# alibaba/EasyParallelLibrary

Hardware: AMD Instinct MI355X
Metric: samples_per_sec (higher is better)
Workload: dtype bf16; 1 GPU; model=bert-large, global_batch=128, seq_len=512, parallelism=dp1

## Files before the change

### csrc/bindings.hip

```cpp

#include <hip/hip_runtime.h>
#include <torch/extension.h>
#include <ATen/hip/impl/HIPStreamMasqueradingAsCUDA.h>

#include <cstdint>

namespace epl {
void register_comm(py::module& m);
}

extern "C" {
void epl_fused_adamw(float*, unsigned short*, const void*, bool, float*,
                     float*, int64_t, float, float, float, float, float, int,
                     float, hipStream_t);
void epl_lamb_phase1(const float*, const void*, bool, float*, float*, float*,
                     const int*, float*, float*, int64_t, float, float, float,
                     float, int, float, hipStream_t);
void epl_lamb_phase2(float*, unsigned short*, const float*, const int*,
                     const float*, int64_t, float, hipStream_t);
void epl_layer_norm_fwd(void*, const void*, const void*, void*, const void*,
                        const void*, float*, float*, int64_t, int64_t, float,
                        bool, hipStream_t);
void epl_layer_norm_bwd(void*, float*, float*, const void*, const void*,
                        const void*, const float*, const float*, float*,
                        float*, int64_t, int64_t, int64_t, bool,
                        hipStream_t);
void epl_bias_gelu_fwd(void*, const void*, const void*, int64_t, int64_t,
                       bool, hipStream_t);
void epl_bias_gelu_bwd(void*, float*, const void*, const void*, const void*,
                       float*, int64_t, int64_t, int64_t, bool,
                       hipStream_t);
void epl_ce_rowstats(const void*, const int64_t*, float*, float*, float*,
                     int64_t, int64_t, int64_t, int64_t, bool, hipStream_t);
void epl_ce_backward(void*, const void*, const int64_t*, const float*,
                     const float*, const float*, int64_t, int64_t, int64_t,
                     int64_t, float, bool, hipStream_t);
void epl_scale(void*, int64_t, float, bool, hipStream_t);
void epl_f32_to_bf16(unsigned short*, const float*, int64_t, hipStream_t);
void epl_bf16_to_f32(float*, const unsigned short*, int64_t, hipStream_t);
void epl_sqnorm(const void*, int64_t, float*, bool, hipStream_t);
void epl_colsum(void*, const void*, float*, int64_t, int64_t, int64_t,
                bool, hipStream_t);
void run_mfma_probe(const unsigned short*, const unsigned short*, float*,
                    hipStream_t);
void epl_moe_dispatch_fwd(void*, const void*, const int64_t*,
                          const int64_t*, const int64_t*, int64_t, int64_t,
                          int64_t, hipStream_t);
void epl_moe_dispatch_bwd(void*, const void*, const int64_t*,
                          const int64_t*, const int64_t*, int64_t, int64_t,
                          int64_t, int64_t, hipStream_t);
void epl_moe_combine_fwd(void*, const void*, const float*, const int64_t*,
                         const int64_t*, const int64_t*, int64_t, int64_t,
                         int64_t, int64_t, hipStream_t);
void epl_moe_combine_bwd(void*, float*, const void*, const void*,
                         const float*, const int64_t*, const int64_t*,
                         const int64_t*, int64_t, int64_t, int64_t,
                         hipStream_t);
void epl_attn_fwd(const void*, const void*, const void*, void*, float*,
                  int64_t, int64_t, float, bool, int64_t, int64_t,
                  const int64_t*,
                  const int64_t*, unsigned int*, int64_t,
                  unsigned long long, int, float, hipStream_t);
void epl_attn_bwd(const void*, const void*, const void*, const void*,
                  const void*, const float*, float*, void*, void*, void*,
                  int64_t, int64_t, float, bool, int64_t, const int64_t*,
                  const int64_t*, const int64_t*, const int64_t*, int,
                  const unsigned int*, int64_t, float, int64_t,
                  const float*, hipStream_t);
}

namespace {

hipStream_t cur_stream() {
  return c10::hip::getCurrentHIPStreamMasqueradingAsCUDA().stream();
}

void check(const at::Tensor& t, at::ScalarType dtype, const char* name) {
  TORCH_CHECK(t.is_cuda(), name, " must be a device tensor");
  TORCH_CHECK(t.is_contiguous(), name, " must be contiguous");
  TORCH_CHECK(t.scalar_type() == dtype, name, " has dtype ", t.scalar_type(),
              ", expected ", dtype);
}

bool is_bf16(const at::Tensor& t) {
  TORCH_CHECK(t.scalar_type() == at::kBFloat16 || t.scalar_type() == at::kFloat,
              "expected bf16 or fp32, got ", t.scalar_type());
  return t.scalar_type() == at::kBFloat16;
}

void fused_adamw(at::Tensor master, c10::optional<at::Tensor> param_bf16,
                 at::Tensor grad, at::Tensor m, at::Tensor v, double lr,
                 double beta1, double beta2, double eps, double weight_decay,
                 int64_t step, double inv_scale) {
  check(master, at::kFloat, "master");
  check(m, at::kFloat, "m");
  check(v, at::kFloat, "v");
  const bool gbf = is_bf16(grad);
  unsigned short* pb = nullptr;
  if (param_bf16.has_value()) {
    check(*param_bf16, at::kBFloat16, "param_bf16");
    TORCH_CHECK(param_bf16->numel() == master.numel());
    pb = reinterpret_cast<unsigned short*>(param_bf16->data_ptr());
  }
  const int64_t n = master.numel();
  TORCH_CHECK(grad.numel() == n && m.numel() == n && v.numel() == n,
              "arena size mismatch");
  epl_fused_adamw(master.data_ptr<float>(), pb, grad.data_ptr(), gbf,
                  m.data_ptr<float>(), v.data_ptr<float>(), n, (float)lr,
                  (float)beta1, (float)beta2, (float)eps, (float)weight_decay,
                  (int)step, (float)inv_scale, cur_stream());
}

void lamb_phase1(at::Tensor master, at::Tensor grad, at::Tensor m,
                 at::Tensor v, at::Tensor update, at::Tensor chunk_of,
                 at::Tensor wnorm_sq, at::Tensor unorm_sq, double beta1,
                 double beta2, double eps, double weight_decay, int64_t step,
                 double inv_scale) {
  check(master, at::kFloat, "master");
  check(update, at::kFloat, "update");
  check(chunk_of, at::kInt, "chunk_of");
  const bool gbf = is_bf16(grad);
  epl_lamb_phase1(master.data_ptr<float>(), grad.data_ptr(), gbf,
                  m.data_ptr<float>(), v.data_ptr<float>(),
                  update.data_ptr<float>(), chunk_of.data_ptr<int>(),
                  wnorm_sq.data_ptr<float>(), unorm_sq.data_ptr<float>(),
                  master.numel(), (float)beta1, (float)beta2, (float)eps,
                  (float)weight_decay, (int)step, (float)inv_scale,
                  cur_stream());
}

void lamb_phase2(at::Tensor master, c10::optional<at::Tensor> param_bf16,
                 at::Tensor update, at::Tensor chunk_of, at::Tensor ratio,
                 double lr) {
  check(master, at::kFloat, "master");
  unsigned short* pb = nullptr;
  if (param_bf16.has_value())
    pb = reinterpret_cast<unsigned short*>(param_bf16->data_ptr());
  epl_lamb_phase2(master.data_ptr<float>(), pb, update.data_ptr<float>(),
                  chunk_of.data_ptr<int>(), ratio.data_ptr<float>(),
                  master.numel(), (float)lr, cur_stream());
}

void layer_norm_fwd(at::Tensor out, at::Tensor x,
                    c10::optional<at::Tensor> res,
                    c10::optional<at::Tensor> sum_out, at::Tensor gamma,
                    at::Tensor beta, at::Tensor mean, at::Tensor rstd,
                    double eps) {
  const bool bf16 = is_bf16(x);
  const int64_t cols = x.size(-1);
  const int64_t rows = x.numel() / cols;
  TORCH_CHECK(!bf16 || cols % 8 == 0, "bf16 LayerNorm needs cols % 8 == 0");
  check(mean, at::kFloat, "mean");
  check(rstd, at::kFloat, "rstd");
  const void* res_p = nullptr;
  void* sum_p = nullptr;
  if (res.has_value()) {
    TORCH_CHECK(sum_out.has_value(),
                "fused residual LayerNorm needs sum_out");
    TORCH_CHECK(res->numel() == x.numel() && sum_out->numel() == x.numel());
    res_p = res->data_ptr();
    sum_p = sum_out->data_ptr();
  }
  epl_layer_norm_fwd(out.data_ptr(), x.data_ptr(), res_p, sum_p,
                     gamma.data_ptr(), beta.data_ptr(),
                     mean.data_ptr<float>(), rstd.data_ptr<float>(), rows,
                     cols, (float)eps, bf16, cur_stream());
}

void layer_norm_bwd(at::Tensor dx, at::Tensor dgamma, at::Tensor dbeta,
                    at::Tensor dy, at::Tensor x, at::Tensor gamma,
                    at::Tensor mean, at::Tensor rstd) {
  const bool bf16 = is_bf16(x);
  const int64_t cols = x.size(-1);
  const int64_t rows = x.numel() / cols;
  TORCH_CHECK(!bf16 || cols % 8 == 0, "bf16 LayerNorm needs cols % 8 == 0");
  TORCH_CHECK((size_t)cols * 2 * sizeof(float) <= 128 * 1024,
              "LayerNorm backward supports cols <= 16384");
  check(dgamma, at::kFloat, "dgamma");
  check(dbeta, at::kFloat, "dbeta");
  float* dgp = nullptr;
  float* dbp = nullptr;
  at::Tensor ws;
  const bool fast = bf16 && cols % 8 == 0 && cols <= 2048;
  int64_t nparts = 0;
  if (fast) {
    const int64_t wave_rows = (rows + 3) / 4;
    nparts = (wave_rows < 1024 ? wave_rows : 1024) * 4;
    ws = at::empty({2, nparts, cols}, dgamma.options());
    dgp = ws.data_ptr<float>();
    dbp = dgp + nparts * cols;
  }
  epl_layer_norm_bwd(dx.data_ptr(), dgamma.data_ptr<float>(),
                     dbeta.data_ptr<float>(), dy.data_ptr(), x.data_ptr(),
                     gamma.data_ptr(), mean.data_ptr<float>(),
                     rstd.data_ptr<float>(), dgp, dbp, nparts, rows, cols,
                     bf16, cur_stream());
}

void bias_gelu_fwd(at::Tensor out, at::Tensor x, at::Tensor bias) {
  const bool bf16 = is_bf16(x);
  const int64_t cols = x.size(-1);
  const int64_t rows = x.numel() / cols;
  TORCH_CHECK(!bf16 || cols % 8 == 0, "bf16 bias_gelu needs cols % 8 == 0");
  epl_bias_gelu_fwd(out.data_ptr(), x.data_ptr(), bias.data_ptr(), rows, cols,
                    bf16, cur_stream());
}

void bias_gelu_bwd(at::Tensor dx, at::Tensor dbias, at::Tensor dy,
                   at::Tensor x, at::Tensor bias) {
  const bool bf16 = is_bf16(x);
  const int64_t cols = x.size(-1);
  const int64_t rows = x.numel() / cols;
  TORCH_CHECK(!bf16 || cols % 8 == 0, "bf16 bias_gelu needs cols % 8 == 0");
  TORCH_CHECK((size_t)cols * sizeof(float) <= 128 * 1024,
              "bias_gelu backward supports cols <= 32768");
  check(dbias, at::kFloat, "dbias");
  float* dbp = nullptr;
  int64_t nwaves = 0;
  at::Tensor ws;
  if (bf16 && cols % 512 == 0) {
    const int64_t segs = cols / 512;
    int64_t per_seg = rows < 1024 ? rows : 1024;
    per_seg = (per_seg + 3) / 4 * 4;
    nwaves = segs * per_seg;
    ws = at::empty({nwaves, 512}, dbias.options());
    dbp = ws.data_ptr<float>();
  }
  epl_bias_gelu_bwd(dx.data_ptr(), dbias.data_ptr<float>(), dy.data_ptr(),
                    x.data_ptr(), bias.data_ptr(), dbp, nwaves, rows, cols,
                    bf16, cur_stream());
}

void ce_rowstats(at::Tensor logits, at::Tensor targets, at::Tensor row_max,
                 at::Tensor row_sumexp, at::Tensor target_logit,
                 int64_t vocab_begin, int64_t ignore_index) {
  const bool bf16 = is_bf16(logits);
  const int64_t cols = logits.size(-1);
  const int64_t rows = logits.numel() / cols;
  check(targets, at::kLong, "targets");
  epl_ce_rowstats(logits.data_ptr(), targets.data_ptr<int64_t>(),
                  row_max.data_ptr<float>(), row_sumexp.data_ptr<float>(),
                  target_logit.data_ptr<float>(), rows, cols, vocab_begin,
                  ignore_index, bf16, cur_stream());
}

void ce_backward(at::Tensor dlogits, at::Tensor logits, at::Tensor targets,
                 at::Tensor gmax, at::Tensor gsumexp, at::Tensor dloss,
                 int64_t vocab_begin, int64_t ignore_index, double scale) {
  const bool bf16 = is_bf16(logits);
  const int64_t cols = logits.size(-1);
  const int64_t rows = logits.numel() / cols;
  epl_ce_backward(dlogits.data_ptr(), logits.data_ptr(),
                  targets.data_ptr<int64_t>(), gmax.data_ptr<float>(),
                  gsumexp.data_ptr<float>(), dloss.data_ptr<float>(), rows,
                  cols, vocab_begin, ignore_index, (float)scale, bf16,
                  cur_stream());
}

void scale_(at::Tensor t, double s) {
  const bool bf16 = is_bf16(t);
  epl_scale(t.data_ptr(), t.numel(), (float)s, bf16, cur_stream());
}

void f32_to_bf16(at::Tensor dst, at::Tensor src) {
  check(dst, at::kBFloat16, "dst");
  check(src, at::kFloat, "src");
  TORCH_CHECK(dst.numel() == src.numel());
  epl_f32_to_bf16(reinterpret_cast<unsigned short*>(dst.data_ptr()),
                  src.data_ptr<float>(), src.numel(), cur_stream());
}

void bf16_to_f32(at::Tensor dst, at::Tensor src) {
  check(dst, at::kFloat, "dst");
  check(src, at::kBFloat16, "src");
  TORCH_CHECK(dst.numel() == src.numel());
  epl_bf16_to_f32(dst.data_ptr<float>(),
                  reinterpret_cast<unsigned short*>(src.data_ptr()),
                  src.numel(), cur_stream());
}

static void attn_strides(const at::Tensor& t, int64_t* out3,
                         const char* name) {
  TORCH_CHECK(t.dim() == 4 && (t.size(3) == 64 || t.size(3) == 128), name,
              " must be [B,H,S,64|128]");
  TORCH_CHECK(t.stride(3) == 1, name, " last dim must be contiguous");
  TORCH_CHECK(t.stride(2) % 8 == 0 && t.stride(1) % 8 == 0,
              name, " row strides must be 16-byte aligned");
  out3[0] = t.stride(0);
  out3[1] = t.stride(1);
  out3[2] = t.stride(2);
}

void attn_fwd(at::Tensor q, at::Tensor k, at::Tensor v, at::Tensor out,
              at::Tensor lse, double scale, bool causal,
              c10::optional<at::Tensor> drop_mask, int64_t seed,
              int64_t drop_thresh, double inv_keep) {
  TORCH_CHECK(q.is_cuda() && q.scalar_type() == at::kBFloat16);
  int64_t in_s[3], o_s[3], tmp[3];
  attn_strides(q, in_s, "q");
  attn_strides(k, tmp, "k");
  TORCH_CHECK(tmp[0] == in_s[0] && tmp[1] == in_s[1] && tmp[2] == in_s[2],
              "q/k/v must share strides");
  attn_strides(v, tmp, "v");
  TORCH_CHECK(tmp[0] == in_s[0] && tmp[1] == in_s[1] && tmp[2] == in_s[2],
              "q/k/v must share strides");
  attn_strides(out, o_s, "out");
  check(lse, at::kFloat, "lse");
  const int64_t heads = q.size(1);
  const int64_t seq = q.size(2);
  const int64_t head_dim = q.size(3);
  const int64_t bh = q.size(0) * heads;
  unsigned int* mptr = nullptr;
  int64_t mask_w = (seq + 31) / 32;
  if (drop_mask.has_value()) {
    check(*drop_mask, at::kInt, "drop_mask");
    TORCH_CHECK(drop_mask->numel() == bh * seq * mask_w,
                "drop_mask size mismatch");
    TORCH_CHECK(drop_thresh > 0 && drop_thresh < 256, "drop_thresh range");
    mptr = reinterpret_cast<unsigned int*>(drop_mask->data_ptr());
  }
  epl_attn_fwd(q.data_ptr(), k.data_ptr(), v.data_ptr(), out.data_ptr(),
               lse.data_ptr<float>(), bh, seq, (float)scale, causal, heads,
               head_dim, in_s, o_s, mptr, mask_w,
               (unsigned long long)seed, (int)drop_thresh,
               (float)inv_keep, cur_stream());
}

void attn_bwd(at::Tensor q, at::Tensor k, at::Tensor v, at::Tensor out,
              at::Tensor dout, at::Tensor lse, at::Tensor delta_ws,
              at::Tensor dq, at::Tensor dk, at::Tensor dv, double scale,
              bool causal, bool split_dkdv,
              c10::optional<at::Tensor> drop_mask, double inv_keep,
              c10::optional<at::Tensor> dlse) {
  int64_t in_s[3], o_s[3], do_s[3], g_s[3], tmp[3];
  attn_strides(q, in_s, "q");
  attn_strides(out, o_s, "out");
  attn_strides(dout, do_s, "dout");
  attn_strides(dq, g_s, "dq");
  attn_strides(dk, tmp, "dk");
  TORCH_CHECK(tmp[0] == g_s[0] && tmp[1] == g_s[1] && tmp[2] == g_s[2],
              "dq/dk/dv must share strides");
  attn_strides(dv, tmp, "dv");
  TORCH_CHECK(tmp[0] == g_s[0] && tmp[1] == g_s[1] && tmp[2] == g_s[2],
              "dq/dk/dv must share strides");
  const int64_t heads = q.size(1);
  const int64_t seq = q.size(2);
  const int64_t bh = q.size(0) * heads;
  check(delta_ws, at::kFloat, "delta_ws");
  const unsigned int* mptr = nullptr;
  int64_t mask_w = (seq + 31) / 32;
  if (drop_mask.has_value()) {
    check(*drop_mask, at::kInt, "drop_mask");
    mptr = reinterpret_cast<const unsigned int*>(drop_mask->data_ptr());
  }
  const float* dlse_ptr = nullptr;
  if (dlse.has_value()) {
    check(*dlse, at::kFloat, "dlse");
    TORCH_CHECK(dlse->numel() == bh * seq, "dlse size mismatch");
    dlse_ptr = dlse->data_ptr<float>();
  }
  epl_attn_bwd(q.data_ptr(), k.data_ptr(), v.data_ptr(), out.data_ptr(),
               dout.data_ptr(), lse.data_ptr<float>(),
               delta_ws.data_ptr<float>(), dq.data_ptr(), dk.data_ptr(),
               dv.data_ptr(), bh, seq, (float)scale, causal, heads, in_s,
               o_s, do_s, g_s, split_dkdv ? 1 : 0, mptr, mask_w,
               (float)inv_keep, q.size(3), dlse_ptr, cur_stream());
}

void mfma_probe(at::Tensor A, at::Tensor B, at::Tensor D) {
  check(A, at::kBFloat16, "A");
  check(B, at::kBFloat16, "B");
  check(D, at::kFloat, "D");
  run_mfma_probe(reinterpret_cast<const unsigned short*>(A.data_ptr()),
                 reinterpret_cast<const unsigned short*>(B.data_ptr()),
                 D.data_ptr<float>(), cur_stream());
}

static void check_idx(const at::Tensor& t, const char* name) {
  TORCH_CHECK(t.is_cuda() && t.is_contiguous() &&
              t.scalar_type() == at::kLong, name,
              " must be a contiguous int64 device tensor");
}

void moe_dispatch_fwd(at::Tensor disp, at::Tensor x, at::Tensor fe,
                      at::Tensor pos, at::Tensor ft, int64_t cap) {
  check(disp, at::kBFloat16, "disp");
  check(x, at::kBFloat16, "x");
  check_idx(fe, "fe"); check_idx(pos, "pos"); check_idx(ft, "ft");
  const int64_t hidden = x.size(-1);
  TORCH_CHECK(hidden % 8 == 0, "hidden % 8");
  epl_moe_dispatch_fwd(disp.data_ptr(), x.data_ptr(),
                       fe.data_ptr<int64_t>(), pos.data_ptr<int64_t>(),
                       ft.data_ptr<int64_t>(), fe.numel(), hidden, cap,
                       cur_stream());
}

void moe_dispatch_bwd(at::Tensor dx, at::Tensor ddisp, at::Tensor fe,
                      at::Tensor pos, at::Tensor inv, int64_t k,
                      int64_t cap) {
  check(dx, at::kBFloat16, "dx");
  check(ddisp, at::kBFloat16, "ddisp");
  check_idx(fe, "fe"); check_idx(pos, "pos"); check_idx(inv, "inv");
  const int64_t hidden = dx.size(-1);
  epl_moe_dispatch_bwd(dx.data_ptr(), ddisp.data_ptr(),
                       fe.data_ptr<int64_t>(), pos.data_ptr<int64_t>(),
                       inv.data_ptr<int64_t>(), dx.numel() / hidden, k,
                       hidden, cap, cur_stream());
}

void moe_combine_fwd(at::Tensor out, at::Tensor h, at::Tensor fw,
                     at::Tensor fe, at::Tensor pos, at::Tensor inv,
                     int64_t k, int64_t cap) {
  check(out, at::kBFloat16, "out");
  check(h, at::kBFloat16, "h");
  check(fw, at::kFloat, "fw");
  check_idx(fe, "fe"); check_idx(pos, "pos"); check_idx(inv, "inv");
  const int64_t hidden = out.size(-1);
  epl_moe_combine_fwd(out.data_ptr(), h.data_ptr(), fw.data_ptr<float>(),
                      fe.data_ptr<int64_t>(), pos.data_ptr<int64_t>(),
                      inv.data_ptr<int64_t>(), out.numel() / hidden, k,
                      hidden, cap, cur_stream());
}

void moe_combine_bwd(at::Tensor dh, at::Tensor dfw, at::Tensor dout,
                     at::Tensor h, at::Tensor fw, at::Tensor fe,
                     at::Tensor pos, at::Tensor ft, int64_t cap) {
  check(dh, at::kBFloat16, "dh");
  check(dout, at::kBFloat16, "dout");
  check(h, at::kBFloat16, "h");
  check(fw, at::kFloat, "fw");
  check(dfw, at::kFloat, "dfw");
  check_idx(fe, "fe"); check_idx(pos, "pos"); check_idx(ft, "ft");
  const int64_t hidden = dh.size(-1);
  epl_moe_combine_bwd(dh.data_ptr(), dfw.data_ptr<float>(),
                      dout.data_ptr(), h.data_ptr(), fw.data_ptr<float>(),
                      fe.data_ptr<int64_t>(), pos.data_ptr<int64_t>(),
                      ft.data_ptr<int64_t>(), fe.numel(), hidden, cap,
                      cur_stream());
}

void colsum(at::Tensor dy, at::Tensor db, at::Tensor partial) {
  const bool bf16 = is_bf16(dy);
  TORCH_CHECK(dy.is_cuda() && dy.is_contiguous() && dy.dim() == 2,
              "dy must be a contiguous 2-D device tensor");
  const int64_t rows = dy.size(0), cols = dy.size(1);
  TORCH_CHECK(cols % 8 == 0, "cols must be a multiple of 8");
  TORCH_CHECK(db.numel() == cols && db.scalar_type() == dy.scalar_type());
  const int64_t stripes = partial.numel() / cols;
  TORCH_CHECK(stripes >= 1 && partial.scalar_type() == at::kFloat);
  epl_colsum(db.data_ptr(), dy.data_ptr(), partial.data_ptr<float>(), rows,
             cols, stripes, bf16, cur_stream());
}

void sqnorm(at::Tensor t, at::Tensor out) {
  const bool bf16 = is_bf16(t);
  check(out, at::kFloat, "out");
  epl_sqnorm(t.data_ptr(), t.numel(), out.data_ptr<float>(), bf16,
             cur_stream());
}

}

PYBIND11_MODULE(TORCH_EXTENSION_NAME, m) {
  m.doc() = "MI355X-native parallel library: RCCL comm core + CDNA4 kernels";
  epl::register_comm(m);
  m.def("fused_adamw", &fused_adamw);
  m.def("colsum", &colsum);
  m.def("lamb_phase1", &lamb_phase1);
  m.def("lamb_phase2", &lamb_phase2);
  m.def("layer_norm_fwd", &layer_norm_fwd);
  m.def("layer_norm_bwd", &layer_norm_bwd);
  m.def("bias_gelu_fwd", &bias_gelu_fwd);
  m.def("bias_gelu_bwd", &bias_gelu_bwd);
  m.def("ce_rowstats", &ce_rowstats);
  m.def("ce_backward", &ce_backward);
  m.def("scale_", &scale_);
  m.def("f32_to_bf16", &f32_to_bf16);
  m.def("bf16_to_f32", &bf16_to_f32);
  m.def("sqnorm", &sqnorm);
  m.def("mfma_probe", &mfma_probe);
  m.def("moe_dispatch_fwd", &moe_dispatch_fwd);
  m.def("moe_dispatch_bwd", &moe_dispatch_bwd);
  m.def("moe_combine_fwd", &moe_combine_fwd);
  m.def("moe_combine_bwd", &moe_combine_bwd);
  m.def("attn_fwd", &attn_fwd);
  m.def("attn_bwd", &attn_bwd);
}
```

### csrc/kernels/attention.hip

```cpp

#include <hip/hip_runtime.h>
#include <cstdint>

using bf16x8 = __attribute__((ext_vector_type(8))) short;
using bf16x4 = __attribute__((ext_vector_type(4))) short;
using f32x16 = __attribute__((ext_vector_type(16))) float;
using i32x2 = __attribute__((ext_vector_type(2))) int;

#define DEVI __device__ __forceinline__

namespace {

DEVI float bf2f(short u) {
  union { unsigned int i; float f; } v;
  v.i = ((unsigned int)(unsigned short)u) << 16;
  return v.f;
}

DEVI unsigned short f2bf(float f) {
  union { float f; unsigned int i; } v;
  v.f = f;
  unsigned int lsb = (v.i >> 16) & 1u;
  return (unsigned short)((v.i + 0x7fffu + lsb) >> 16);
}

DEVI unsigned int pack2(float a, float b) {
  return (unsigned int)f2bf(a) | ((unsigned int)f2bf(b) << 16);
}

DEVI int crow(int r, int hi) {
  return (r & 3) + 8 * (r >> 2) + 4 * hi;
}

DEVI bf16x8 assemble_pfrag(const float* p) {
  unsigned int c0 = pack2(p[0], p[1]);
  unsigned int c1 = pack2(p[2], p[3]);
  unsigned int c2 = pack2(p[4], p[5]);
  unsigned int c3 = pack2(p[6], p[7]);
  i32x2 r = __builtin_amdgcn_permlane32_swap((int)c0, (int)c2, false, false);
  i32x2 s = __builtin_amdgcn_permlane32_swap((int)c1, (int)c3, false, false);
  union { unsigned int d[4]; bf16x8 v; } out;
  out.d[0] = (unsigned int)r[0];
  out.d[1] = (unsigned int)s[0];
  out.d[2] = (unsigned int)r[1];
  out.d[3] = (unsigned int)s[1];
  return out.v;
}

DEVI void philox_round(unsigned int& c0, unsigned int& c1,
                       unsigned int& c2, unsigned int& c3,
                       unsigned int k0, unsigned int k1) {
  const unsigned int hi0 = __umulhi(0xD2511F53u, c0);
  const unsigned int lo0 = 0xD2511F53u * c0;
  const unsigned int hi1 = __umulhi(0xCD9E8D57u, c2);
  const unsigned int lo1 = 0xCD9E8D57u * c2;
  c0 = hi1 ^ c1 ^ k0;
  c1 = lo1;
  c2 = hi0 ^ c3 ^ k1;
  c3 = lo0;
}

DEVI void philox4x32(unsigned int c0, unsigned int c1, unsigned int c2,
                     unsigned int c3, unsigned int k0, unsigned int k1,
                     unsigned int out[4]) {
#pragma unroll
  for (int i = 0; i < 10; ++i) {
    philox_round(c0, c1, c2, c3, k0, k1);
    k0 += 0x9E3779B9u;
    k1 += 0xBB67AE85u;
  }
  out[0] = c0; out[1] = c1; out[2] = c2; out[3] = c3;
}


template <bool MASKED, bool DROP, int D>
DEVI void fwd_tile(const short (&ldsK)[64][D + 8],
                   const short (&ldsV)[D][72],
                   int sub, int64_t kvs, int64_t seq, int64_t myq,
                   float scale, int causal, const bf16x8 (&qfrag)[D / 16],
                   f32x16 (&ot)[D / 32], float& m, float& l, int lq,
                   int hi, unsigned int* maskrow, int64_t mask_w,
                   unsigned int seed0, unsigned int seed1,
                   unsigned int bh32, int drop_thresh, float inv_keep) {
  f32x16 st = {};
#pragma unroll
  for (int c = 0; c < D / 16; ++c) {
    bf16x8 kfrag =
        *reinterpret_cast<const bf16x8*>(&ldsK[sub + lq][hi * 8 + 16 * c]);
    st = __builtin_amdgcn_mfma_f32_32x32x16_bf16(kfrag, qfrag[c], st, 0, 0,
                                                 0);
  }
  float s[16];
  float tile_max = -1e30f;
#pragma unroll
  for (int r = 0; r < 16; ++r) {
    float sv = st[r] * scale;
    if (MASKED) {
      const int64_t kvg = kvs + crow(r, hi);
      if (kvg >= seq || (causal && kvg > myq)) sv = -1e30f;
    }
    s[r] = sv;
    tile_max = fmaxf(tile_max, sv);
  }
  tile_max = fmaxf(tile_max, __shfl_xor(tile_max, 32, 64));
  const float m_new = fmaxf(m, tile_max);
  const float alpha = __expf(m - m_new);
  float rowsum = 0.f;
#pragma unroll
  for (int r = 0; r < 16; ++r) {
    s[r] = __expf(s[r] - m_new);
    rowsum += s[r];
  }
  rowsum += __shfl_xor(rowsum, 32, 64);
  l = l * alpha + rowsum;
  m = m_new;
  if (DROP) {
    unsigned int rnd[4];
    philox4x32((unsigned int)myq,
               (unsigned int)(kvs >> 5) * 2u + (unsigned int)hi,
               bh32, 0x2E1B2137u, seed0, seed1, rnd);
    unsigned int mybits = 0;
#pragma unroll
    for (int r = 0; r < 16; ++r) {
      const unsigned int byte = (rnd[r >> 2] >> ((r & 3) * 8)) & 0xFFu;
      const bool keep = (int)byte >= drop_thresh;
      s[r] = keep ? s[r] * inv_keep : 0.f;
      mybits |= (unsigned int)keep << crow(r, hi);
    }
    const unsigned int word = mybits | __shfl_xor(mybits, 32, 64);
    if (hi == 0 && myq < seq)
      maskrow[myq * mask_w + (kvs >> 5)] = word;
  }
#pragma unroll
  for (int j = 0; j < D / 32; ++j)
#pragma unroll
    for (int r = 0; r < 16; ++r)
      ot[j][r] *= alpha;
  bf16x8 pf0 = assemble_pfrag(&s[0]);
  bf16x8 pf1 = assemble_pfrag(&s[8]);
#pragma unroll
  for (int kc = 0; kc < 2; ++kc) {
    bf16x8 pf = kc == 0 ? pf0 : pf1;
#pragma unroll
    for (int j = 0; j < D / 32; ++j) {
      bf16x8 vt = *reinterpret_cast<const bf16x8*>(
          &ldsV[j * 32 + lq][sub + kc * 16 + hi * 8]);
      ot[j] = __builtin_amdgcn_mfma_f32_32x32x16_bf16(vt, pf, ot[j], 0, 0,
                                                      0);
    }
  }
}

template <bool DROP, int D>
__global__ __launch_bounds__(256, D == 64 ? 3 : 2) void attn_fwd_kernel(
    const short* __restrict__ q, const short* __restrict__ k,
    const short* __restrict__ v, short* __restrict__ out,
    float* __restrict__ lse, int64_t seq, float scale, int causal,
    int64_t heads, int64_t in_sb, int64_t in_sh, int64_t in_ss,
    int64_t o_sb, int64_t o_sh, int64_t o_ss,
    unsigned int* __restrict__ mask, int64_t mask_w,
    unsigned long long seed, int drop_thresh, float inv_keep) {
  __shared__ short ldsV[2][D][72];
  __shared__ short ldsK[2][64][D + 8];
  const int lane = threadIdx.x & 63;
  const int wave = threadIdx.x >> 6;
  const int hi = lane >> 5;
  const int lq = lane & 31;
  const int64_t bh = causal ? (int64_t)blockIdx.x : (int64_t)blockIdx.y;
  const int64_t boff = (bh / heads) * in_sb + (bh % heads) * in_sh;
  const int64_t qb = causal ? (int64_t)gridDim.y - 1 - blockIdx.y
                            : (int64_t)blockIdx.x;
  const int64_t q0_blk = qb * 128;
  const int64_t q0 = q0_blk + wave * 32;
  const bool active = q0 < seq;
  const short* qp = q + boff;
  const short* kp = k + boff;
  const short* vp = v + boff;

  const int64_t myq = q0 + lq;
  const int64_t qrow = myq < seq ? myq : seq - 1;

  bf16x8 qfrag[D / 16];
#pragma unroll
  for (int c = 0; c < D / 16; ++c)
    qfrag[c] = *reinterpret_cast<const bf16x8*>(
        qp + qrow * in_ss + hi * 8 + 16 * c);

  f32x16 ot[D / 32] = {};
  float m = -1e30f, l = 0.f;

  const int64_t bulk_end = causal ? q0_blk : (seq & ~(int64_t)63);
  const int64_t blk_kv_end =
      causal ? (q0_blk + 128 < seq ? q0_blk + 128 : seq) : seq;
  const int stage_kv = threadIdx.x & 63;
  const int stage_d0 = (threadIdx.x >> 6) * 8;

  bf16x8 pv[D / 32], pk[D / 32];
  auto load_tile = [&](int64_t kv0) {
    int64_t vrow = kv0 + stage_kv;
    if (vrow >= seq) vrow = seq - 1;
#pragma unroll
    for (int h2 = 0; h2 < D / 32; ++h2) {
      const int sd = stage_d0 + h2 * 32;
      pv[h2] = *reinterpret_cast<const bf16x8*>(vp + vrow * in_ss + sd);
      pk[h2] = *reinterpret_cast<const bf16x8*>(kp + vrow * in_ss + sd);
    }
  };
  auto write_tile = [&](int b) {
#pragma unroll
    for (int h2 = 0; h2 < D / 32; ++h2) {
      const int sd = stage_d0 + h2 * 32;
#pragma unroll
      for (int j = 0; j < 8; ++j)
        ldsV[b][sd + j][stage_kv] = pv[h2][j];
      *reinterpret_cast<bf16x8*>(&ldsK[b][stage_kv][sd]) = pk[h2];
    }
  };

  unsigned int* maskrow =
      DROP ? mask + bh * seq * mask_w : (unsigned int*)nullptr;
  const unsigned int seed0 = (unsigned int)seed;
  const unsigned int seed1 = (unsigned int)(seed >> 32);
  const unsigned int bh32 = (unsigned int)bh;

  int buf = 0;
  if (blk_kv_end > 0) load_tile(0);
  int64_t kv0 = 0;
  for (; kv0 < bulk_end; kv0 += 64) {
    write_tile(buf);
    __syncthreads();
    if (kv0 + 64 < blk_kv_end) load_tile(kv0 + 64);
#pragma unroll
    for (int sub = 0; sub < 64; sub += 32)
      fwd_tile<false, DROP, D>(ldsK[buf], ldsV[buf], sub, kv0 + sub, seq,
                               myq, scale, causal, qfrag, ot, m, l, lq,
                               hi, maskrow, mask_w, seed0, seed1, bh32,
                               drop_thresh, inv_keep);
    buf ^= 1;
  }
  for (; kv0 < blk_kv_end; kv0 += 64) {
    write_tile(buf);
    __syncthreads();
    if (kv0 + 64 < blk_kv_end) load_tile(kv0 + 64);
    if (active) {
      const int64_t wave_kv_end = causal
          ? (q0 + 32 < seq ? q0 + 32 : seq) : seq;
#pragma unroll
      for (int sub = 0; sub < 64; sub += 32) {
        const int64_t kvs = kv0 + sub;
        if (kvs >= wave_kv_end) break;
        fwd_tile<true, DROP, D>(ldsK[buf], ldsV[buf], sub, kvs, seq, myq,
                                scale, causal, qfrag, ot, m, l, lq, hi,
                                maskrow, mask_w, seed0, seed1, bh32,
                                drop_thresh, inv_keep);
      }
    }
    buf ^= 1;
  }

  if (!active || myq >= seq) return;
  const float inv_l = 1.f / l;
  short* op = out + (bh / heads) * o_sb + (bh % heads) * o_sh + myq * o_ss;
#pragma unroll
  for (int j = 0; j < D / 32; ++j)
#pragma unroll
    for (int r = 0; r < 16; ++r)
      op[j * 32 + crow(r, hi)] = (short)f2bf(ot[j][r] * inv_l);
  if (hi == 0) lse[bh * seq + myq] = m + __logf(l);
}

__global__ void attn_bwd_prep_kernel(const short* __restrict__ dout,
                                     const short* __restrict__ out,
                                     float* __restrict__ delta,
                                     int64_t rows, int64_t seq,
                                     int64_t heads, int64_t do_sb,
                                     int64_t do_sh, int64_t do_ss,
                                     int64_t o_sb, int64_t o_sh,
                                     int64_t o_ss) {
  const int lane = threadIdx.x & 63;
  const int waves_per_block = blockDim.x >> 6;
  for (int64_t row = (int64_t)blockIdx.x * waves_per_block +
                     (threadIdx.x >> 6);
       row < rows; row += (int64_t)gridDim.x * waves_per_block) {
    const int64_t bh = row / seq;
    const int64_t sq = row % seq;
    const short* dp = dout + (bh / heads) * do_sb + (bh % heads) * do_sh +
                      sq * do_ss;
    const short* op = out + (bh / heads) * o_sb + (bh % heads) * o_sh +
                      sq * o_ss;
    float acc = bf2f(dp[lane]) * bf2f(op[lane]);
#pragma unroll
    for (int off = 32; off > 0; off >>= 1)
      acc += __shfl_down(acc, off, 64);
    if (lane == 0) delta[row] = acc;
  }
}

__global__ __launch_bounds__(256) void attn_bwd_dkdv_kernel(
    const short* __restrict__ q, const short* __restrict__ k,
    const short* __restrict__ v, const short* __restrict__ dout,
    const float* __restrict__ lse, const float* __restrict__ delta,
    short* __restrict__ dk, short* __restrict__ dv, int64_t seq,
    float scale, int causal, int64_t heads, int64_t in_sb, int64_t in_sh,
    int64_t in_ss, int64_t do_sb, int64_t do_sh, int64_t do_ss,
    int64_t g_sb, int64_t g_sh, int64_t g_ss) {
  __shared__ short ldsQ[32][72];
  __shared__ short ldsDO[32][72];
  const int lane = threadIdx.x & 63;
  const int wave = threadIdx.x >> 6;
  const int hi = lane >> 5;
  const int lkv = lane & 31;
  const int64_t bh = blockIdx.y;
  const int64_t kv0_blk = (int64_t)blockIdx.x * 128;
  const int64_t kv0 = kv0_blk + wave * 32;
  const bool active = kv0 < seq;
  const int64_t boff = (bh / heads) * in_sb + (bh % heads) * in_sh;
  const short* qp = q + boff;
  const short* kp = k + boff;
  const short* vp = v + boff;
  const short* dop = dout + (bh / heads) * do_sb + (bh % heads) * do_sh;
  const float* lsep = lse + bh * seq;
  const float* dltp = delta + bh * seq;

  const int64_t mykv = kv0 + lkv;
  const int64_t kvrow = mykv < seq ? mykv : seq - 1;

  bf16x8 kfrag[4], vfrag[4];
#pragma unroll
  for (int c = 0; c < 4; ++c) {
    kfrag[c] = *reinterpret_cast<const bf16x8*>(
        kp + kvrow * in_ss + hi * 8 + 16 * c);
    vfrag[c] = *reinterpret_cast<const bf16x8*>(
        vp + kvrow * in_ss + hi * 8 + 16 * c);
  }

  f32x16 dvt0 = {}, dvt1 = {};
  f32x16 dkt0 = {}, dkt1 = {};

  const int stage_row = threadIdx.x >> 3;
  const int stage_seg = (threadIdx.x & 7) * 8;
  const int64_t q_start = causal ? (kv0_blk / 32) * 32 : 0;
  for (int64_t q0 = q_start; q0 < seq; q0 += 32) {
    __syncthreads();
    {
      int64_t qr = q0 + stage_row;
      if (qr >= seq) qr = seq - 1;
      *reinterpret_cast<bf16x8*>(&ldsQ[stage_row][stage_seg]) =
          *reinterpret_cast<const bf16x8*>(qp + qr * in_ss + stage_seg);
      *reinterpret_cast<bf16x8*>(&ldsDO[stage_row][stage_seg]) =
          *reinterpret_cast<const bf16x8*>(dop + qr * do_ss + stage_seg);
    }
    __syncthreads();
    if (!active || (causal && q0 + 31 < kv0)) continue;
    f32x16 st = {};
    f32x16 dpt = {};
#pragma unroll
    for (int c = 0; c < 4; ++c) {
      bf16x8 qf = *reinterpret_cast<const bf16x8*>(
          &ldsQ[lkv][hi * 8 + 16 * c]);
      bf16x8 dof = *reinterpret_cast<const bf16x8*>(
          &ldsDO[lkv][hi * 8 + 16 * c]);
      st = __builtin_amdgcn_mfma_f32_32x32x16_bf16(qf, kfrag[c], st, 0, 0,
                                                   0);
      dpt = __builtin_amdgcn_mfma_f32_32x32x16_bf16(dof, vfrag[c], dpt, 0,
                                                    0, 0);
    }
    float p[16], ds[16];
#pragma unroll
    for (int r = 0; r < 16; ++r) {
      const int64_t qg = q0 + crow(r, hi);
      const int64_t qgc = qg < seq ? qg : seq - 1;
      float sv = st[r] * scale;
      bool masked = qg >= seq || (causal && mykv > qg) || mykv >= seq;
      float pv = masked ? 0.f : __expf(sv - lsep[qgc]);
      p[r] = pv;
      ds[r] = masked ? 0.f : pv * (dpt[r] - dltp[qgc]) * scale;
    }
    bf16x8 pb0 = assemble_pfrag(&p[0]);
    bf16x8 pb1 = assemble_pfrag(&p[8]);
    bf16x8 db0 = assemble_pfrag(&ds[0]);
    bf16x8 db1 = assemble_pfrag(&ds[8]);
#pragma unroll
    for (int qc = 0; qc < 2; ++qc) {
      bf16x8 dot0, dot1, qt0, qt1;
#pragma unroll
      for (int j = 0; j < 8; ++j) {
        const int qr = qc * 16 + hi * 8 + j;
        dot0[j] = ldsDO[qr][lkv];
        dot1[j] = ldsDO[qr][32 + lkv];
        qt0[j] = ldsQ[qr][lkv];
        qt1[j] = ldsQ[qr][32 + lkv];
      }
      bf16x8 pb = qc == 0 ? pb0 : pb1;
      bf16x8 db = qc == 0 ? db0 : db1;
      dvt0 = __builtin_amdgcn_mfma_f32_32x32x16_bf16(dot0, pb, dvt0, 0, 0,
                                                     0);
      dvt1 = __builtin_amdgcn_mfma_f32_32x32x16_bf16(dot1, pb, dvt1, 0, 0,
                                                     0);
      dkt0 = __builtin_amdgcn_mfma_f32_32x32x16_bf16(qt0, db, dkt0, 0, 0,
                                                     0);
      dkt1 = __builtin_amdgcn_mfma_f32_32x32x16_bf16(qt1, db, dkt1, 0, 0,
                                                     0);
    }
  }

  if (!active || mykv >= seq) return;
  const int64_t goff = (bh / heads) * g_sb + (bh % heads) * g_sh +
                       mykv * g_ss;
  short* dkp = dk + goff;
  short* dvp = dv + goff;
#pragma unroll
  for (int r = 0; r < 16; ++r) {
    dvp[crow(r, hi)] = (short)f2bf(dvt0[r]);
    dvp[32 + crow(r, hi)] = (short)f2bf(dvt1[r]);
    dkp[crow(r, hi)] = (short)f2bf(dkt0[r]);
    dkp[32 + crow(r, hi)] = (short)f2bf(dkt1[r]);
  }
}


template <bool MASKED, bool DROP, int D>
DEVI void dv_tile(const short (&ldsQ)[64][D + 8],
                  const short (&ldsDO)[64][D + 8],
                  int sub, int64_t q0, int64_t seq, int64_t mykv,
                  float scale, int causal, const float* lsep,
                  const bf16x8 (&kfrag)[D / 16], f32x16 (&dvt)[D / 32],
                  int lkv, int hi, const unsigned int* maskrow,
                  int64_t mask_w, float inv_keep) {
  f32x16 st = {};
#pragma unroll
  for (int c = 0; c < D / 16; ++c) {
    bf16x8 qf = *reinterpret_cast<const bf16x8*>(
        &ldsQ[sub + lkv][hi * 8 + 16 * c]);
    st = __builtin_amdgcn_mfma_f32_32x32x16_bf16(qf, kfrag[c], st, 0, 0, 0);
  }
  float p[16];
#pragma unroll
  for (int r = 0; r < 16; ++r) {
    const int64_t qg = q0 + crow(r, hi);
    const int64_t qgc = qg < seq ? qg : seq - 1;
    if (MASKED) {
      bool masked = qg >= seq || (causal && mykv > qg) || mykv >= seq;
      p[r] = masked ? 0.f : __expf(st[r] * scale - lsep[qgc]);
    } else {
      p[r] = __expf(st[r] * scale - lsep[qg]);
    }
    if (DROP) {
      const int64_t kvc = mykv < seq ? mykv : seq - 1;
      const unsigned int w = maskrow[qgc * mask_w + (kvc >> 5)];
      p[r] *= ((w >> (kvc & 31)) & 1u) ? inv_keep : 0.f;
    }
  }
  bf16x8 pb0 = assemble_pfrag(&p[0]);
  bf16x8 pb1 = assemble_pfrag(&p[8]);
#pragma unroll
  for (int qc = 0; qc < 2; ++qc) {
    bf16x8 pb = qc == 0 ? pb0 : pb1;
#pragma unroll
    for (int dj = 0; dj < D / 32; ++dj) {
      bf16x8 dot;
#pragma unroll
      for (int j = 0; j < 8; ++j) {
        const int qr = sub + qc * 16 + hi * 8 + j;
        dot[j] = ldsDO[qr][dj * 32 + lkv];
      }
      dvt[dj] =
          __builtin_amdgcn_mfma_f32_32x32x16_bf16(dot, pb, dvt[dj], 0, 0, 0);
    }
  }
}

template <bool MASKED, bool DROP, int D>
DEVI void dk_tile(const short (&ldsQ)[64][D + 8],
                  const short (&ldsDO)[64][D + 8],
                  int sub, int64_t q0, int64_t seq, int64_t mykv,
                  float scale, int causal, const float* lsep,
                  const float* dltp, const bf16x8 (&kfrag)[D / 16],
                  const bf16x8 (&vfrag)[D / 16], f32x16 (&dkt)[D / 32],
                  int lkv, int hi, const unsigned int* maskrow,
                  int64_t mask_w, float inv_keep) {
  f32x16 st = {};
  f32x16 dpt = {};
#pragma unroll
  for (int c = 0; c < D / 16; ++c) {
    bf16x8 qf = *reinterpret_cast<const bf16x8*>(
        &ldsQ[sub + lkv][hi * 8 + 16 * c]);
    bf16x8 dof = *reinterpret_cast<const bf16x8*>(
        &ldsDO[sub + lkv][hi * 8 + 16 * c]);
    st = __builtin_amdgcn_mfma_f32_32x32x16_bf16(qf, kfrag[c], st, 0, 0, 0);
    dpt = __builtin_amdgcn_mfma_f32_32x32x16_bf16(dof, vfrag[c], dpt, 0, 0,
                                                  0);
  }
  float ds[16];
#pragma unroll
  for (int r = 0; r < 16; ++r) {
    const int64_t qg = q0 + crow(r, hi);
    const int64_t qgc = qg < seq ? qg : seq - 1;
    float dp = dpt[r];
    if (DROP) {
      const int64_t kvc = mykv < seq ? mykv : seq - 1;
      const unsigned int w = maskrow[qgc * mask_w + (kvc >> 5)];
      dp *= ((w >> (kvc & 31)) & 1u) ? inv_keep : 0.f;
    }
    if (MASKED) {
      bool masked = qg >= seq || (causal && mykv > qg) || mykv >= seq;
      float pv = masked ? 0.f : __expf(st[r] * scale - lsep[qgc]);
      ds[r] = masked ? 0.f : pv * (dp - dltp[qgc]) * scale;
    } else {
      float pv = __expf(st[r] * scale - lsep[qg]);
      ds[r] = pv * (dp - dltp[qg]) * scale;
    }
  }
  bf16x8 db0 = assemble_pfrag(&ds[0]);
  bf16x8 db1 = assemble_pfrag(&ds[8]);
#pragma unroll
  for (int qc = 0; qc < 2; ++qc) {
    bf16x8 db = qc == 0 ? db0 : db1;
#pragma unroll
    for (int dj = 0; dj < D / 32; ++dj) {
      bf16x8 qt;
#pragma unroll
      for (int j = 0; j < 8; ++j) {
        const int qr = sub + qc * 16 + hi * 8 + j;
        qt[j] = ldsQ[qr][dj * 32 + lkv];
      }
      dkt[dj] =
          __builtin_amdgcn_mfma_f32_32x32x16_bf16(qt, db, dkt[dj], 0, 0, 0);
    }
  }
}

template <bool DROP, bool DBUF, int D>
__global__ __launch_bounds__(256, D == 64 ? (DBUF ? 3 : 4) : 2)
void attn_bwd_dv_kernel(
    const short* __restrict__ q, const short* __restrict__ k,
    const short* __restrict__ dout, const float* __restrict__ lse,
    short* __restrict__ dv, int64_t seq, float scale, int causal,
    int64_t heads, int64_t in_sb, int64_t in_sh, int64_t in_ss,
    int64_t do_sb, int64_t do_sh, int64_t do_ss, int64_t g_sb,
    int64_t g_sh, int64_t g_ss,
    const unsigned int* __restrict__ mask, int64_t mask_w,
    float inv_keep) {
  __shared__ short ldsQ[DBUF ? 2 : 1][64][D + 8];
  __shared__ short ldsDO[DBUF ? 2 : 1][64][D + 8];
  const int lane = threadIdx.x & 63;
  const int wave = threadIdx.x >> 6;
  const int hi = lane >> 5;
  const int lkv = lane & 31;
  const int64_t bh = causal ? (int64_t)blockIdx.x : (int64_t)blockIdx.y;
  const int64_t kv0_blk =
      (causal ? (int64_t)blockIdx.y : (int64_t)blockIdx.x) * 128;
  const int64_t kv0 = kv0_blk + wave * 32;
  const bool active = kv0 < seq;
  const int64_t boff = (bh / heads) * in_sb + (bh % heads) * in_sh;
  const short* qp = q + boff;
  const short* kp = k + boff;
  const short* dop = dout + (bh / heads) * do_sb + (bh % heads) * do_sh;
  const float* lsep = lse + bh * seq;

  const int64_t mykv = kv0 + lkv;
  const int64_t kvrow = mykv < seq ? mykv : seq - 1;
  bf16x8 kfrag[D / 16];
#pragma unroll
  for (int c = 0; c < D / 16; ++c)
    kfrag[c] = *reinterpret_cast<const bf16x8*>(
        kp + kvrow * in_ss + hi * 8 + 16 * c);

  f32x16 dvt[D / 32] = {};
  const int stage_row = threadIdx.x >> 3;
  const int stage_seg = (threadIdx.x & 7) * 8;

  bf16x8 rq[2][D / 64], rdo[2][D / 64];
  auto prefetch = [&](int64_t q0) {
#pragma unroll
    for (int half = 0; half < 2; ++half) {
      int64_t qr = q0 + stage_row + half * 32;
      if (qr >= seq) qr = seq - 1;
#pragma unroll
      for (int s = 0; s < D / 64; ++s) {
        rq[half][s] = *reinterpret_cast<const bf16x8*>(
            qp + qr * in_ss + stage_seg + s * 64);
        rdo[half][s] = *reinterpret_cast<const bf16x8*>(
            dop + qr * do_ss + stage_seg + s * 64);
      }
    }
  };
  auto commit = [&](int buf) {
#pragma unroll
    for (int half = 0; half < 2; ++half)
#pragma unroll
      for (int s = 0; s < D / 64; ++s) {
        *reinterpret_cast<bf16x8*>(
            &ldsQ[buf][stage_row + half * 32][stage_seg + s * 64]) =
            rq[half][s];
        *reinterpret_cast<bf16x8*>(
            &ldsDO[buf][stage_row + half * 32][stage_seg + s * 64]) =
            rdo[half][s];
      }
  };
  auto stage_q64 = [&](int64_t q0) {
    __syncthreads();
#pragma unroll
    for (int half = 0; half < 2; ++half) {
      int64_t qr = q0 + stage_row + half * 32;
      if (qr >= seq) qr = seq - 1;
#pragma unroll
      for (int seg = 0; seg < D; seg += 64) {
        *reinterpret_cast<bf16x8*>(
            &ldsQ[0][stage_row + half * 32][stage_seg + seg]) =
            *reinterpret_cast<const bf16x8*>(
                qp + qr * in_ss + stage_seg + seg);
        *reinterpret_cast<bf16x8*>(
            &ldsDO[0][stage_row + half * 32][stage_seg + seg]) =
            *reinterpret_cast<const bf16x8*>(
                dop + qr * do_ss + stage_seg + seg);
      }
    }
    __syncthreads();
  };

  const unsigned int* maskrow =
      DROP ? mask + bh * seq * mask_w : (const unsigned int*)nullptr;
  const int64_t diag_end =
      causal ? (kv0_blk + 128 < seq ? kv0_blk + 128 : seq) : 0;
  const int64_t bulk_end = seq & ~(int64_t)63;
  if (!DBUF) {
    int64_t q0 = causal ? kv0_blk : 0;
    for (; q0 < diag_end; q0 += 64) {
      stage_q64(q0);
      if (!active) continue;
#pragma unroll
      for (int sub = 0; sub < 64; sub += 32) {
        const int64_t q0s = q0 + sub;
        if (q0s >= diag_end || (causal && q0s + 31 < kv0)) continue;
        dv_tile<true, DROP, D>(ldsQ[0], ldsDO[0], sub, q0s, seq, mykv,
                               scale, causal, lsep, kfrag, dvt, lkv, hi,
                               maskrow, mask_w, inv_keep);
      }
    }
    q0 = diag_end > q0 ? diag_end : q0;
    for (; q0 + 63 < bulk_end; q0 += 64) {
      stage_q64(q0);
#pragma unroll
      for (int sub = 0; sub < 64; sub += 32)
        dv_tile<false, DROP, D>(ldsQ[0], ldsDO[0], sub, q0 + sub, seq,
                                mykv, scale, causal, lsep, kfrag, dvt,
                                lkv, hi, maskrow, mask_w, inv_keep);
    }
    for (; q0 < seq; q0 += 64) {
      stage_q64(q0);
      if (!active) continue;
#pragma unroll
      for (int sub = 0; sub < 64; sub += 32) {
        const int64_t q0s = q0 + sub;
        if (q0s >= seq) break;
        dv_tile<true, DROP, D>(ldsQ[0], ldsDO[0], sub, q0s, seq, mykv,
                               scale, causal, lsep, kfrag, dvt, lkv, hi,
                               maskrow, mask_w, inv_keep);
      }
    }
  } else {
    const int64_t q_begin = causal ? kv0_blk : 0;
    int buf = 0;
    prefetch(q_begin);
    for (int64_t q0 = q_begin; q0 < seq; q0 += 64) {
      commit(buf);
      __syncthreads();
      if (q0 + 64 < seq) prefetch(q0 + 64);
      const int rb = buf;
      buf ^= 1;
      const bool plain = q0 >= diag_end && q0 + 63 < bulk_end;
      if (plain) {
#pragma unroll
        for (int sub = 0; sub < 64; sub += 32)
          dv_tile<false, DROP, D>(ldsQ[rb], ldsDO[rb], sub, q0 + sub,
                                  seq, mykv, scale, causal, lsep, kfrag,
                                  dvt, lkv, hi, maskrow, mask_w,
                                  inv_keep);
      } else if (active) {
#pragma unroll
        for (int sub = 0; sub < 64; sub += 32) {
          const int64_t q0s = q0 + sub;
          if (q0s >= seq) break;
          if (causal && q0s + 31 < kv0) continue;
          dv_tile<true, DROP, D>(ldsQ[rb], ldsDO[rb], sub, q0s, seq,
                                 mykv, scale, causal, lsep, kfrag, dvt,
                                 lkv, hi, maskrow, mask_w, inv_keep);
        }
      }
    }
  }
  if (!active || mykv >= seq) return;
  short* dvp = dv + (bh / heads) * g_sb + (bh % heads) * g_sh +
               mykv * g_ss;
#pragma unroll
  for (int dj = 0; dj < D / 32; ++dj)
#pragma unroll
    for (int r = 0; r < 16; ++r)
      dvp[dj * 32 + crow(r, hi)] = (short)f2bf(dvt[dj][r]);
}

template <bool DROP, bool DBUF, int D>
__global__ __launch_bounds__(256, D == 64 ? 3 : 2) void attn_bwd_dk_kernel(
    const short* __restrict__ q, const short* __restrict__ k,
    const short* __restrict__ v, const short* __restrict__ dout,
    const float* __restrict__ lse, const float* __restrict__ delta,
    short* __restrict__ dk, int64_t seq, float scale, int causal,
    int64_t heads, int64_t in_sb, int64_t in_sh, int64_t in_ss,
    int64_t do_sb, int64_t do_sh, int64_t do_ss, int64_t g_sb,
    int64_t g_sh, int64_t g_ss,
    const unsigned int* __restrict__ mask, int64_t mask_w,
    float inv_keep) {
  __shared__ short ldsQ[DBUF ? 2 : 1][64][D + 8];
  __shared__ short ldsDO[DBUF ? 2 : 1][64][D + 8];
  const int lane = threadIdx.x & 63;
  const int wave = threadIdx.x >> 6;
  const int hi = lane >> 5;
  const int lkv = lane & 31;
  const int64_t bh = causal ? (int64_t)blockIdx.x : (int64_t)blockIdx.y;
  const int64_t kv0_blk =
      (causal ? (int64_t)blockIdx.y : (int64_t)blockIdx.x) * 128;
  const int64_t kv0 = kv0_blk + wave * 32;
  const bool active = kv0 < seq;
  const int64_t boff = (bh / heads) * in_sb + (bh % heads) * in_sh;
  const short* qp = q + boff;
  const short* kp = k + boff;
  const short* vp = v + boff;
  const short* dop = dout + (bh / heads) * do_sb + (bh % heads) * do_sh;
  const float* lsep = lse + bh * seq;
  const float* dltp = delta + bh * seq;

  const int64_t mykv = kv0 + lkv;
  const int64_t kvrow = mykv < seq ? mykv : seq - 1;
  bf16x8 kfrag[D / 16], vfrag[D / 16];
#pragma unroll
  for (int c = 0; c < D / 16; ++c) {
    kfrag[c] = *reinterpret_cast<const bf16x8*>(
        kp + kvrow * in_ss + hi * 8 + 16 * c);
    vfrag[c] = *reinterpret_cast<const bf16x8*>(
        vp + kvrow * in_ss + hi * 8 + 16 * c);
  }

  f32x16 dkt[D / 32] = {};
  const int stage_row = threadIdx.x >> 3;
  const int stage_seg = (threadIdx.x & 7) * 8;

  bf16x8 rq[2][D / 64], rdo[2][D / 64];
  auto prefetch = [&](int64_t q0) {
#pragma unroll
    for (int half = 0; half < 2; ++half) {
      int64_t qr = q0 + stage_row + half * 32;
      if (qr >= seq) qr = seq - 1;
#pragma unroll
      for (int s = 0; s < D / 64; ++s) {
        rq[half][s] = *reinterpret_cast<const bf16x8*>(
            qp + qr * in_ss + stage_seg + s * 64);
        rdo[half][s] = *reinterpret_cast<const bf16x8*>(
            dop + qr * do_ss + stage_seg + s * 64);
      }
    }
  };
  auto commit = [&](int buf) {
#pragma unroll
    for (int half = 0; half < 2; ++half)
#pragma unroll
      for (int s = 0; s < D / 64; ++s) {
        *reinterpret_cast<bf16x8*>(
            &ldsQ[buf][stage_row + half * 32][stage_seg + s * 64]) =
            rq[half][s];
        *reinterpret_cast<bf16x8*>(
            &ldsDO[buf][stage_row + half * 32][stage_seg + s * 64]) =
            rdo[half][s];
      }
  };
  auto stage_q64 = [&](int64_t q0) {
    __syncthreads();
#pragma unroll
    for (int half = 0; half < 2; ++half) {
      int64_t qr = q0 + stage_row + half * 32;
      if (qr >= seq) qr = seq - 1;
#pragma unroll
      for (int seg = 0; seg < D; seg += 64) {
        *reinterpret_cast<bf16x8*>(
            &ldsQ[0][stage_row + half * 32][stage_seg + seg]) =
            *reinterpret_cast<const bf16x8*>(
                qp + qr * in_ss + stage_seg + seg);
        *reinterpret_cast<bf16x8*>(
            &ldsDO[0][stage_row + half * 32][stage_seg + seg]) =
            *reinterpret_cast<const bf16x8*>(
                dop + qr * do_ss + stage_seg + seg);
      }
    }
    __syncthreads();
  };

  const unsigned int* maskrow =
      DROP ? mask + bh * seq * mask_w : (const unsigned int*)nullptr;
  const int64_t diag_end =
      causal ? (kv0_blk + 128 < seq ? kv0_blk + 128 : seq) : 0;
  const int64_t bulk_end = seq & ~(int64_t)63;
  if (!DBUF) {
    int64_t q0 = causal ? kv0_blk : 0;
    for (; q0 < diag_end; q0 += 64) {
      stage_q64(q0);
      if (!active) continue;
#pragma unroll
      for (int sub = 0; sub < 64; sub += 32) {
        const int64_t q0s = q0 + sub;
        if (q0s >= diag_end || (causal && q0s + 31 < kv0)) continue;
        dk_tile<true, DROP, D>(ldsQ[0], ldsDO[0], sub, q0s, seq, mykv,
                               scale, causal, lsep, dltp, kfrag, vfrag,
                               dkt, lkv, hi, maskrow, mask_w, inv_keep);
      }
    }
    q0 = diag_end > q0 ? diag_end : q0;
    for (; q0 + 63 < bulk_end; q0 += 64) {
      stage_q64(q0);
#pragma unroll
      for (int sub = 0; sub < 64; sub += 32)
        dk_tile<false, DROP, D>(ldsQ[0], ldsDO[0], sub, q0 + sub, seq,
                                mykv, scale, causal, lsep, dltp, kfrag,
                                vfrag, dkt, lkv, hi, maskrow, mask_w,
                                inv_keep);
    }
    for (; q0 < seq; q0 += 64) {
      stage_q64(q0);
      if (!active) continue;
#pragma unroll
      for (int sub = 0; sub < 64; sub += 32) {
        const int64_t q0s = q0 + sub;
        if (q0s >= seq) break;
        dk_tile<true, DROP, D>(ldsQ[0], ldsDO[0], sub, q0s, seq, mykv,
                               scale, causal, lsep, dltp, kfrag, vfrag,
                               dkt, lkv, hi, maskrow, mask_w, inv_keep);
      }
    }
  } else {
    const int64_t q_begin = causal ? kv0_blk : 0;
    int buf = 0;
    prefetch(q_begin);
    for (int64_t q0 = q_begin; q0 < seq; q0 += 64) {
      commit(buf);
      __syncthreads();
      if (q0 + 64 < seq) prefetch(q0 + 64);
      const int rb = buf;
      buf ^= 1;
      const bool plain = q0 >= diag_end && q0 + 63 < bulk_end;
      if (plain) {
#pragma unroll
        for (int sub = 0; sub < 64; sub += 32)
          dk_tile<false, DROP, D>(ldsQ[rb], ldsDO[rb], sub, q0 + sub,
                                  seq, mykv, scale, causal, lsep, dltp,
                                  kfrag, vfrag, dkt, lkv, hi, maskrow,
                                  mask_w, inv_keep);
      } else if (active) {
#pragma unroll
        for (int sub = 0; sub < 64; sub += 32) {
          const int64_t q0s = q0 + sub;
          if (q0s >= seq) break;
          if (causal && q0s + 31 < kv0) continue;
          dk_tile<true, DROP, D>(ldsQ[rb], ldsDO[rb], sub, q0s, seq,
                                 mykv, scale, causal, lsep, dltp, kfrag,
                                 vfrag, dkt, lkv, hi, maskrow, mask_w,
                                 inv_keep);
        }
      }
    }
  }
  if (!active || mykv >= seq) return;
  short* dkp = dk + (bh / heads) * g_sb + (bh % heads) * g_sh +
               mykv * g_ss;
#pragma unroll
  for (int dj = 0; dj < D / 32; ++dj)
#pragma unroll
    for (int r = 0; r < 16; ++r)
      dkp[dj * 32 + crow(r, hi)] = (short)f2bf(dkt[dj][r]);
}


template <bool MASKED, bool DROP, int D>
DEVI void dq_tile(const short (&ldsK)[64][D + 8],
                  const short (&ldsVr)[64][D + 8],
                  int sub, int64_t kv0, int64_t seq, int64_t myq,
                  float scale, int causal, float mylse, float mydelta,
                  const bf16x8 (&qfrag)[D / 16],
                  const bf16x8 (&dofrag)[D / 16],
                  f32x16 (&dqt)[D / 32], int lq, int hi,
                  const unsigned int* maskrow, int64_t mask_w,
                  float inv_keep) {
  f32x16 st = {};
  f32x16 dpt = {};
#pragma unroll
  for (int c = 0; c < D / 16; ++c) {
    bf16x8 kf = *reinterpret_cast<const bf16x8*>(
        &ldsK[sub + lq][hi * 8 + 16 * c]);
    bf16x8 vf = *reinterpret_cast<const bf16x8*>(
        &ldsVr[sub + lq][hi * 8 + 16 * c]);
    st = __builtin_amdgcn_mfma_f32_32x32x16_bf16(kf, qfrag[c], st, 0, 0, 0);
    dpt = __builtin_amdgcn_mfma_f32_32x32x16_bf16(vf, dofrag[c], dpt, 0, 0,
                                                  0);
  }
  unsigned int mword = 0;
  if (DROP) {
    const int64_t qc = myq < seq ? myq : seq - 1;
    mword = maskrow[qc * mask_w + (kv0 >> 5)];
  }
  float ds[16];
#pragma unroll
  for (int r = 0; r < 16; ++r) {
    float pv = __expf(st[r] * scale - mylse);
    if (MASKED) {
      const int64_t kvg = kv0 + crow(r, hi);
      if (myq >= seq || kvg >= seq || (causal && kvg > myq)) pv = 0.f;
    }
    float dp = dpt[r];
    if (DROP)
      dp *= ((mword >> crow(r, hi)) & 1u) ? inv_keep : 0.f;
    ds[r] = pv * (dp - mydelta) * scale;
  }
  bf16x8 db0 = assemble_pfrag(&ds[0]);
  bf16x8 db1 = assemble_pfrag(&ds[8]);
#pragma unroll
  for (int kc = 0; kc < 2; ++kc) {
    bf16x8 db = kc == 0 ? db0 : db1;
#pragma unroll
    for (int dj = 0; dj < D / 32; ++dj) {
      bf16x8 kt;
#pragma unroll
      for (int j = 0; j < 8; ++j) {
        const int kr = sub + kc * 16 + hi * 8 + j;
        kt[j] = ldsK[kr][dj * 32 + lq];
      }
      dqt[dj] =
          __builtin_amdgcn_mfma_f32_32x32x16_bf16(kt, db, dqt[dj], 0, 0, 0);
    }
  }
}

template <bool DROP, bool DBUF, int D>
__global__ __launch_bounds__(256, D == 64 ? 3 : 2) void attn_bwd_dq_kernel(
    const short* __restrict__ q, const short* __restrict__ k,
    const short* __restrict__ v, const short* __restrict__ dout,
    const float* __restrict__ lse, const float* __restrict__ delta,
    short* __restrict__ dq, const short* __restrict__ out, int64_t seq,
    float scale, int causal, int64_t heads, int64_t in_sb, int64_t in_sh,
    int64_t in_ss, int64_t do_sb, int64_t do_sh, int64_t do_ss,
    int64_t g_sb, int64_t g_sh, int64_t g_ss, int64_t o_sb, int64_t o_sh,
    int64_t o_ss, const unsigned int* __restrict__ mask, int64_t mask_w,
    float inv_keep, const float* __restrict__ dlse) {
  __shared__ short ldsK[DBUF ? 2 : 1][64][D + 8];
  __shared__ short ldsVr[DBUF ? 2 : 1][64][D + 8];
  const int lane = threadIdx.x & 63;
  const int wave = threadIdx.x >> 6;
  const int hi = lane >> 5;
  const int lq = lane & 31;
  const int64_t bh = causal ? (int64_t)blockIdx.x : (int64_t)blockIdx.y;
  const int64_t qb = causal ? (int64_t)gridDim.y - 1 - blockIdx.y
                            : (int64_t)blockIdx.x;
  const int64_t q0_blk = qb * 128;
  const int64_t q0 = q0_blk + wave * 32;
  const bool active = q0 < seq;
  const int64_t boff = (bh / heads) * in_sb + (bh % heads) * in_sh;
  const short* qp = q + boff;
  const short* kp = k + boff;
  const short* vp = v + boff;
  const short* dop = dout + (bh / heads) * do_sb + (bh % heads) * do_sh;

  const int64_t myq = q0 + lq;
  const int64_t qrow = myq < seq ? myq : seq - 1;
  const float mylse = lse[bh * seq + qrow];

  const short* op_ = out + (bh / heads) * o_sb + (bh % heads) * o_sh;
  bf16x8 qfrag[D / 16], dofrag[D / 16];
  float dsum = 0.f;
#pragma unroll
  for (int c = 0; c < D / 16; ++c) {
    qfrag[c] = *reinterpret_cast<const bf16x8*>(
        qp + qrow * in_ss + hi * 8 + 16 * c);
    dofrag[c] = *reinterpret_cast<const bf16x8*>(
        dop + qrow * do_ss + hi * 8 + 16 * c);
    bf16x8 of = *reinterpret_cast<const bf16x8*>(
        op_ + qrow * o_ss + hi * 8 + 16 * c);
#pragma unroll
    for (int j = 0; j < 8; ++j)
      dsum += bf2f(dofrag[c][j]) * bf2f(of[j]);
  }
  float mydelta = dsum + __shfl_xor(dsum, 32, 64);
  if (dlse != nullptr) mydelta -= dlse[bh * seq + qrow];
  if (myq < seq && hi == 0)
    const_cast<float*>(delta)[bh * seq + myq] = mydelta;

  f32x16 dqt[D / 32] = {};

  const int stage_row = threadIdx.x >> 3;
  const int stage_seg = (threadIdx.x & 7) * 8;
  const int64_t bulk_end = causal ? q0_blk : (seq & ~(int64_t)63);
  const int64_t blk_kv_end =
      causal ? (q0_blk + 128 < seq ? q0_blk + 128 : seq) : seq;

  auto stage_kv64 = [&](int64_t kv0) {
    __syncthreads();
#pragma unroll
    for (int half = 0; half < 2; ++half) {
      int64_t kr = kv0 + stage_row + half * 32;
      if (kr >= seq) kr = seq - 1;
#pragma unroll
      for (int seg = 0; seg < D; seg += 64) {
        *reinterpret_cast<bf16x8*>(
            &ldsK[0][stage_row + half * 32][stage_seg + seg]) =
            *reinterpret_cast<const bf16x8*>(
                kp + kr * in_ss + stage_seg + seg);
        *reinterpret_cast<bf16x8*>(
            &ldsVr[0][stage_row + half * 32][stage_seg + seg]) =
            *reinterpret_cast<const bf16x8*>(
                vp + kr * in_ss + stage_seg + seg);
      }
    }
    __syncthreads();
  };

  bf16x8 rk[2][D / 64], rv[2][D / 64];
  auto prefetch = [&](int64_t kv0) {
#pragma unroll
    for (int half = 0; half < 2; ++half) {
      int64_t kr = kv0 + stage_row + half * 32;
      if (kr >= seq) kr = seq - 1;
#pragma unroll
      for (int s = 0; s < D / 64; ++s) {
        rk[half][s] = *reinterpret_cast<const bf16x8*>(
            kp + kr * in_ss + stage_seg + s * 64);
        rv[half][s] = *reinterpret_cast<const bf16x8*>(
            vp + kr * in_ss + stage_seg + s * 64);
      }
    }
  };
  auto commit = [&](int buf) {
#pragma unroll
    for (int half = 0; half < 2; ++half)
#pragma unroll
      for (int s = 0; s < D / 64; ++s) {
        *reinterpret_cast<bf16x8*>(
            &ldsK[buf][stage_row + half * 32][stage_seg + s * 64]) =
            rk[half][s];
        *reinterpret_cast<bf16x8*>(
            &ldsVr[buf][stage_row + half * 32][stage_seg + s * 64]) =
            rv[half][s];
      }
  };

  const unsigned int* maskrow =
      DROP ? mask + bh * seq * mask_w : (const unsigned int*)nullptr;
  if (!DBUF) {
    int64_t kv0 = 0;
    for (; kv0 < bulk_end; kv0 += 64) {
      stage_kv64(kv0);
#pragma unroll
      for (int sub = 0; sub < 64; sub += 32)
        dq_tile<false, DROP, D>(ldsK[0], ldsVr[0], sub, kv0 + sub, seq,
                                myq, scale, causal, mylse, mydelta,
                                qfrag, dofrag, dqt, lq, hi, maskrow,
                                mask_w, inv_keep);
    }
    for (; kv0 < blk_kv_end; kv0 += 64) {
      stage_kv64(kv0);
      const int64_t wave_kv_end = causal
          ? (q0 + 32 < seq ? q0 + 32 : seq) : seq;
      if (!active) continue;
#pragma unroll
      for (int sub = 0; sub < 64; sub += 32) {
        const int64_t kvs = kv0 + sub;
        if (kvs >= wave_kv_end) break;
        dq_tile<true, DROP, D>(ldsK[0], ldsVr[0], sub, kvs, seq, myq,
                               scale, causal, mylse, mydelta, qfrag,
                               dofrag, dqt, lq, hi, maskrow, mask_w,
                               inv_keep);
      }
    }
  } else {
    int buf = 0;
    prefetch(0);
    for (int64_t kv0 = 0; kv0 < blk_kv_end; kv0 += 64) {
      commit(buf);
      __syncthreads();
      if (kv0 + 64 < blk_kv_end) prefetch(kv0 + 64);
      const int rb = buf;
      buf ^= 1;
      if (kv0 < bulk_end) {
#pragma unroll
        for (int sub = 0; sub < 64; sub += 32)
          dq_tile<false, DROP, D>(ldsK[rb], ldsVr[rb], sub, kv0 + sub,
                                  seq, myq, scale, causal, mylse,
                                  mydelta, qfrag, dofrag, dqt, lq, hi,
                                  maskrow, mask_w, inv_keep);
      } else if (active) {
        const int64_t wave_kv_end = causal
            ? (q0 + 32 < seq ? q0 + 32 : seq) : seq;
#pragma unroll
        for (int sub = 0; sub < 64; sub += 32) {
          const int64_t kvs = kv0 + sub;
          if (kvs >= wave_kv_end) break;
          dq_tile<true, DROP, D>(ldsK[rb], ldsVr[rb], sub, kvs, seq,
                                 myq, scale, causal, mylse, mydelta,
                                 qfrag, dofrag, dqt, lq, hi, maskrow,
                                 mask_w, inv_keep);
        }
      }
    }
  }

  if (!active || myq >= seq) return;
  short* dqp = dq + (bh / heads) * g_sb + (bh % heads) * g_sh + myq * g_ss;
#pragma unroll
  for (int dj = 0; dj < D / 32; ++dj)
#pragma unroll
    for (int r = 0; r < 16; ++r)
      dqp[dj * 32 + crow(r, hi)] = (short)f2bf(dqt[dj][r]);
}

}

extern "C" {

void epl_attn_fwd(const void* q, const void* k, const void* v, void* out,
                  float* lse, int64_t batch_heads, int64_t seq, float scale,
                  bool causal, int64_t heads, int64_t head_dim,
                  const int64_t* in_strides,
                  const int64_t* o_strides, unsigned int* drop_mask,
                  int64_t mask_w, unsigned long long seed, int drop_thresh,
                  float inv_keep, hipStream_t stream) {
  const unsigned nqb = (unsigned)((seq + 127) / 128);
  dim3 grid = causal ? dim3((unsigned)batch_heads, nqb)
                     : dim3(nqb, (unsigned)batch_heads);
#define FWD_ARGS                                                         \
  reinterpret_cast<const short*>(q), reinterpret_cast<const short*>(k),  \
      reinterpret_cast<const short*>(v), reinterpret_cast<short*>(out),  \
      lse, seq, scale, causal ? 1 : 0, heads, in_strides[0],             \
      in_strides[1], in_strides[2], o_strides[0], o_strides[1],          \
      o_strides[2], drop_mask, mask_w, seed, drop_thresh, inv_keep
  if (head_dim == 128) {
    if (drop_mask != nullptr)
      hipLaunchKernelGGL(HIP_KERNEL_NAME(attn_fwd_kernel<true, 128>),
                         grid, dim3(256), 0, stream, FWD_ARGS);
    else
      hipLaunchKernelGGL(HIP_KERNEL_NAME(attn_fwd_kernel<false, 128>),
                         grid, dim3(256), 0, stream, FWD_ARGS);
  } else if (drop_mask != nullptr) {
    hipLaunchKernelGGL(HIP_KERNEL_NAME(attn_fwd_kernel<true, 64>), grid,
                       dim3(256), 0, stream, FWD_ARGS);
  } else {
    hipLaunchKernelGGL(HIP_KERNEL_NAME(attn_fwd_kernel<false, 64>), grid,
                       dim3(256), 0, stream, FWD_ARGS);
  }
#undef FWD_ARGS
}

void epl_attn_bwd(const void* q, const void* k, const void* v,
                  const void* out, const void* dout, const float* lse,
                  float* delta_ws, void* dq, void* dk, void* dv,
                  int64_t batch_heads, int64_t seq, float scale,
                  bool causal, int64_t heads, const int64_t* in_strides,
                  const int64_t* o_strides, const int64_t* do_strides,
                  const int64_t* g_strides, int split_dkdv,
                  const unsigned int* drop_mask, int64_t mask_w,
                  float inv_keep, int64_t head_dim, const float* dlse,
                  hipStream_t stream) {
  const int64_t rows = batch_heads * seq;
  const unsigned nqb = (unsigned)((seq + 127) / 128);
  dim3 grid = causal ? dim3((unsigned)batch_heads, nqb)
                     : dim3(nqb, (unsigned)batch_heads);
  if (split_dkdv || drop_mask != nullptr || head_dim == 128 || causal ||
      dlse != nullptr) {
#define DV_ARGS                                                          \
  reinterpret_cast<const short*>(q), reinterpret_cast<const short*>(k),  \
      reinterpret_cast<const short*>(dout), lse,                         \
      reinterpret_cast<short*>(dv), seq, scale, causal ? 1 : 0, heads,   \
      in_strides[0], in_strides[1], in_strides[2], do_strides[0],        \
      do_strides[1], do_strides[2], g_strides[0], g_strides[1],          \
      g_strides[2], drop_mask, mask_w, inv_keep
#define DQ_ARGS                                                          \
  reinterpret_cast<const short*>(q), reinterpret_cast<const short*>(k),  \
      reinterpret_cast<const short*>(v),                                 \
      reinterpret_cast<const short*>(dout), lse, delta_ws,               \
      reinterpret_cast<short*>(dq), reinterpret_cast<const short*>(out), \
      seq, scale, causal ? 1 : 0, heads, in_strides[0], in_strides[1],   \
      in_strides[2], do_strides[0], do_strides[1], do_strides[2],        \
      g_strides[0], g_strides[1], g_strides[2], o_strides[0],            \
      o_strides[1], o_strides[2], drop_mask, mask_w, inv_keep, dlse
#define DK_ARGS                                                          \
  reinterpret_cast<const short*>(q), reinterpret_cast<const short*>(k),  \
      reinterpret_cast<const short*>(v),                                 \
      reinterpret_cast<const short*>(dout), lse, delta_ws,               \
      reinterpret_cast<short*>(dk), seq, scale, causal ? 1 : 0, heads,   \
      in_strides[0], in_strides[1], in_strides[2], do_strides[0],        \
      do_strides[1], do_strides[2], g_strides[0], g_strides[1],          \
      g_strides[2], drop_mask, mask_w, inv_keep
    static const int dbuf_mode = [] {
      const char* e = getenv("EPL_ATTN_BWD_DBUF");
      return e == nullptr ? -1 : atoi(e);
    }();
    const int mode = dbuf_mode < 0 ? (causal ? 0 : 2) : dbuf_mode;
    const bool dbuf = mode >= 1;
    const bool dbuf_k = mode >= 2;
    const bool dbuf_q = mode >= 3;
    if (head_dim == 128) {
      if (drop_mask != nullptr) {
        hipLaunchKernelGGL(
            HIP_KERNEL_NAME(attn_bwd_dv_kernel<true, false, 128>), grid,
            dim3(256), 0, stream, DV_ARGS);
        hipLaunchKernelGGL(
            HIP_KERNEL_NAME(attn_bwd_dq_kernel<true, false, 128>), grid,
            dim3(256), 0, stream, DQ_ARGS);
        hipLaunchKernelGGL(
            HIP_KERNEL_NAME(attn_bwd_dk_kernel<true, false, 128>), grid,
            dim3(256), 0, stream, DK_ARGS);
      } else {
        hipLaunchKernelGGL(
            HIP_KERNEL_NAME(attn_bwd_dv_kernel<false, false, 128>), grid,
            dim3(256), 0, stream, DV_ARGS);
        hipLaunchKernelGGL(
            HIP_KERNEL_NAME(attn_bwd_dq_kernel<false, false, 128>), grid,
            dim3(256), 0, stream, DQ_ARGS);
        hipLaunchKernelGGL(
            HIP_KERNEL_NAME(attn_bwd_dk_kernel<false, false, 128>), grid,
            dim3(256), 0, stream, DK_ARGS);
      }
    } else if (drop_mask != nullptr) {
      if (dbuf)
        hipLaunchKernelGGL(
            HIP_KERNEL_NAME(attn_bwd_dv_kernel<true, true, 64>), grid,
            dim3(256), 0, stream, DV_ARGS);
      else
        hipLaunchKernelGGL(
            HIP_KERNEL_NAME(attn_bwd_dv_kernel<true, false, 64>), grid,
            dim3(256), 0, stream, DV_ARGS);
      if (dbuf_q)
        hipLaunchKernelGGL(
            HIP_KERNEL_NAME(attn_bwd_dq_kernel<true, true, 64>), grid,
            dim3(256), 0, stream, DQ_ARGS);
      else
        hipLaunchKernelGGL(
            HIP_KERNEL_NAME(attn_bwd_dq_kernel<true, false, 64>), grid,
            dim3(256), 0, stream, DQ_ARGS);
      if (dbuf_k)
        hipLaunchKernelGGL(
            HIP_KERNEL_NAME(attn_bwd_dk_kernel<true, true, 64>), grid,
            dim3(256), 0, stream, DK_ARGS);
      else
        hipLaunchKernelGGL(
            HIP_KERNEL_NAME(attn_bwd_dk_kernel<true, false, 64>), grid,
            dim3(256), 0, stream, DK_ARGS);
    } else {
      if (dbuf)
        hipLaunchKernelGGL(
            HIP_KERNEL_NAME(attn_bwd_dv_kernel<false, true, 64>), grid,
            dim3(256), 0, stream, DV_ARGS);
      else
        hipLaunchKernelGGL(
            HIP_KERNEL_NAME(attn_bwd_dv_kernel<false, false, 64>), grid,
            dim3(256), 0, stream, DV_ARGS);
      if (dbuf_q)
        hipLaunchKernelGGL(
            HIP_KERNEL_NAME(attn_bwd_dq_kernel<false, true, 64>), grid,
            dim3(256), 0, stream, DQ_ARGS);
      else
        hipLaunchKernelGGL(
            HIP_KERNEL_NAME(attn_bwd_dq_kernel<false, false, 64>), grid,
            dim3(256), 0, stream, DQ_ARGS);
      if (dbuf_k)
        hipLaunchKernelGGL(
            HIP_KERNEL_NAME(attn_bwd_dk_kernel<false, true, 64>), grid,
            dim3(256), 0, stream, DK_ARGS);
      else
        hipLaunchKernelGGL(
            HIP_KERNEL_NAME(attn_bwd_dk_kernel<false, false, 64>), grid,
            dim3(256), 0, stream, DK_ARGS);
    }
#undef DV_ARGS
#undef DQ_ARGS
#undef DK_ARGS
    return;
  }
  {
    const int64_t blocks = (rows + 3) / 4;
    hipLaunchKernelGGL(attn_bwd_prep_kernel,
                       dim3((unsigned)(blocks < 4096 ? blocks : 4096)),
                       dim3(256), 0, stream,
                       reinterpret_cast<const short*>(dout),
                       reinterpret_cast<const short*>(out), delta_ws, rows,
                       seq, heads, do_strides[0], do_strides[1],
                       do_strides[2], o_strides[0], o_strides[1],
                       o_strides[2]);
  }
  hipLaunchKernelGGL(attn_bwd_dkdv_kernel, grid, dim3(256), 0, stream,
                     reinterpret_cast<const short*>(q),
                     reinterpret_cast<const short*>(k),
                     reinterpret_cast<const short*>(v),
                     reinterpret_cast<const short*>(dout), lse, delta_ws,
                     reinterpret_cast<short*>(dk),
                     reinterpret_cast<short*>(dv), seq, scale,
                     causal ? 1 : 0, heads, in_strides[0], in_strides[1],
                     in_strides[2], do_strides[0], do_strides[1],
                     do_strides[2], g_strides[0], g_strides[1],
                     g_strides[2]);
  hipLaunchKernelGGL(HIP_KERNEL_NAME(attn_bwd_dq_kernel<false, false, 64>),
                     grid, dim3(256), 0, stream,
                     reinterpret_cast<const short*>(q),
                     reinterpret_cast<const short*>(k),
                     reinterpret_cast<const short*>(v),
                     reinterpret_cast<const short*>(dout), lse, delta_ws,
                     reinterpret_cast<short*>(dq),
                     reinterpret_cast<const short*>(out), seq, scale,
                     causal ? 1 : 0, heads, in_strides[0], in_strides[1],
                     in_strides[2], do_strides[0], do_strides[1],
                     do_strides[2], g_strides[0], g_strides[1],
                     g_strides[2], o_strides[0], o_strides[1],
                     o_strides[2], drop_mask, mask_w, inv_keep, dlse);
}

}
```

### csrc/kernels/mfma_probe.hip

```cpp

#include <hip/hip_runtime.h>

using bf16x8 = __attribute__((ext_vector_type(8))) short;
using f32x16 = __attribute__((ext_vector_type(16))) float;

__global__ void mfma_probe_kernel(const unsigned short* __restrict__ A,
                                  const unsigned short* __restrict__ B,
                                  float* __restrict__ D) {
  const int lane = threadIdx.x & 63;
  const int half = lane >> 5;
  const int lm = lane & 31;
  bf16x8 a, b;
  for (int j = 0; j < 8; ++j) {
    a[j] = (short)A[lm * 16 + (half * 8 + j)];
    b[j] = (short)B[(half * 8 + j) * 32 + lm];
  }
  f32x16 c = {};
  c = __builtin_amdgcn_mfma_f32_32x32x16_bf16(a, b, c, 0, 0, 0);
  for (int reg = 0; reg < 16; ++reg) {
    const int row = (reg & 3) + 8 * (reg >> 2) + 4 * half;
    const int col = lm;
    D[row * 32 + col] = c[reg];
  }
}

extern "C" void run_mfma_probe(const unsigned short* A,
                               const unsigned short* B, float* D,
                               hipStream_t stream) {
  hipLaunchKernelGGL(mfma_probe_kernel, dim3(1), dim3(64), 0, stream, A, B,
                     D);
}
```

Measured before the change: 634.1 samples/s.

## Use LDS transpose reads and hardware bf16 packing in attention backward kernels

Reworks the attention backward dV/dK/dQ kernels to stage Q and dO in a padded LDS image and read transposed MFMA fragments with ds_read_tr16_b64 instead of per-element gathers. LSE/delta row constants are staged in LDS and preloaded into accumulators, and bf16 packing uses the hardware convert instruction with vectorized stores. The aim is to cut LDS gather instructions and scalar conversion cost in the backward pass. It adds a probe kernel to validate the transpose layout, an env var to fall back to the old tiles, and raises the occupancy hint for head_dim 128 without dropout, which risks register pressure.

Measured after the change: 681.3 samples/s (median of 6 runs). 7.4% higher.

```diff
diff --git a/csrc/bindings.hip b/csrc/bindings.hip
--- a/csrc/bindings.hip
+++ b/csrc/bindings.hip
@@ -43,6 +43,7 @@
                 bool, hipStream_t);
 void run_mfma_probe(const unsigned short*, const unsigned short*, float*,
                     hipStream_t);
+void run_tr_read_probe(short*, short*, int, hipStream_t);
 void epl_moe_dispatch_fwd(void*, const void*, const int64_t*,
                           const int64_t*, const int64_t*, int64_t, int64_t,
                           int64_t, hipStream_t);
@@ -367,6 +368,19 @@
                (float)inv_keep, q.size(3), dlse_ptr, cur_stream());
 }
 
+void tr_read_probe(at::Tensor out_gather, at::Tensor out_tr,
+                   int64_t head_dim) {
+  TORCH_CHECK(head_dim == 64 || head_dim == 128, "head_dim must be 64|128");
+  check(out_gather, at::kShort, "out_gather");
+  check(out_tr, at::kShort, "out_tr");
+  const int64_t n = 4 * (head_dim / 32) * 64 * 8;
+  TORCH_CHECK(out_gather.numel() == n && out_tr.numel() == n,
+              "probe outputs must hold ", n, " elements");
+  run_tr_read_probe(reinterpret_cast<short*>(out_gather.data_ptr()),
+                    reinterpret_cast<short*>(out_tr.data_ptr()),
+                    (int)head_dim, cur_stream());
+}
+
 void mfma_probe(at::Tensor A, at::Tensor B, at::Tensor D) {
   check(A, at::kBFloat16, "A");
   check(B, at::kBFloat16, "B");
@@ -479,6 +493,7 @@
   m.def("bf16_to_f32", &bf16_to_f32);
   m.def("sqnorm", &sqnorm);
   m.def("mfma_probe", &mfma_probe);
+  m.def("tr_read_probe", &tr_read_probe);
   m.def("moe_dispatch_fwd", &moe_dispatch_fwd);
   m.def("moe_dispatch_bwd", &moe_dispatch_bwd);
   m.def("moe_combine_fwd", &moe_combine_fwd);
diff --git a/csrc/kernels/attention.hip b/csrc/kernels/attention.hip
--- a/csrc/kernels/attention.hip
+++ b/csrc/kernels/attention.hip
@@ -1,11 +1,20 @@
 
 #include <hip/hip_runtime.h>
 #include <cstdint>
+#include <cstdlib>
+#include <cstring>
+#include <type_traits>
+
+#include "attn_lds_image.h"
 
 using bf16x8 = __attribute__((ext_vector_type(8))) short;
 using bf16x4 = __attribute__((ext_vector_type(4))) short;
 using f32x16 = __attribute__((ext_vector_type(16))) float;
 using i32x2 = __attribute__((ext_vector_type(2))) int;
+using u32x2 = __attribute__((ext_vector_type(2))) unsigned int;
+using f32x2 = __attribute__((ext_vector_type(2))) float;
+using f32x4 = __attribute__((ext_vector_type(4))) float;
+using bf16v2 = __attribute__((ext_vector_type(2))) __bf16;
 
 #define DEVI __device__ __forceinline__
 
@@ -32,11 +41,18 @@
   return (r & 3) + 8 * (r >> 2) + 4 * hi;
 }
 
+DEVI unsigned int cvt_pk_bf16(float a, float b) {
+  f32x2 f = {a, b};
+  return __builtin_bit_cast(unsigned int,
+                            __builtin_convertvector(f, bf16v2));
+}
+
+template <bool HW = false>
 DEVI bf16x8 assemble_pfrag(const float* p) {
-  unsigned int c0 = pack2(p[0], p[1]);
-  unsigned int c1 = pack2(p[2], p[3]);
-  unsigned int c2 = pack2(p[4], p[5]);
-  unsigned int c3 = pack2(p[6], p[7]);
+  unsigned int c0 = HW ? cvt_pk_bf16(p[0], p[1]) : pack2(p[0], p[1]);
+  unsigned int c1 = HW ? cvt_pk_bf16(p[2], p[3]) : pack2(p[2], p[3]);
+  unsigned int c2 = HW ? cvt_pk_bf16(p[4], p[5]) : pack2(p[4], p[5]);
+  unsigned int c3 = HW ? cvt_pk_bf16(p[6], p[7]) : pack2(p[6], p[7]);
   i32x2 r = __builtin_amdgcn_permlane32_swap((int)c0, (int)c2, false, false);
   i32x2 s = __builtin_amdgcn_permlane32_swap((int)c1, (int)c3, false, false);
   union { unsigned int d[4]; bf16x8 v; } out;
@@ -45,6 +61,49 @@
   out.d[2] = (unsigned int)r[1];
   out.d[3] = (unsigned int)s[1];
   return out.v;
+}
+
+using attn_img::img_off;
+using attn_img::img_pitch;
+using attn_img::tr_frag;
+
+template <bool TR, int D>
+DEVI short* img_at(short (&img)[64][TR ? img_pitch<D>() : D + 8], int row,
+                   int col) {
+  return TR ? &img[0][0] + img_off<D>(row, col >> 3) : &img[row][col];
+}
+
+DEVI f32x16 load_rowconst(const float* c32, int hi) {
+  f32x16 out;
+#pragma unroll
+  for (int g = 0; g < 4; ++g) {
+    const f32x4 v = *reinterpret_cast<const f32x4*>(c32 + 8 * g + 4 * hi);
+    out[4 * g + 0] = v[0];
+    out[4 * g + 1] = v[1];
+    out[4 * g + 2] = v[2];
+    out[4 * g + 3] = v[3];
+  }
+  return out;
+}
+
+struct RowMask {
+  int lo, hi_;
+  DEVI RowMask(int64_t q0, int64_t seq, int64_t mykv, int causal) {
+    const int64_t rows = seq - q0;
+    hi_ = mykv >= seq ? 0 : (rows < 32 ? (int)rows : 32);
+    const int64_t d = mykv - q0;
+    lo = (causal && d > 0) ? (d < 32 ? (int)d : 32) : 0;
+  }
+  DEVI bool masked(int c) const { return c < lo || c >= hi_; }
+};
+
+DEVI void store_acc_bf16(short* p, const f32x16& acc, int hi) {
+#pragma unroll
+  for (int g = 0; g < 4; ++g) {
+    u32x2 v = {cvt_pk_bf16(acc[4 * g], acc[4 * g + 1]),
+               cvt_pk_bf16(acc[4 * g + 2], acc[4 * g + 3])};
+    *reinterpret_cast<u32x2*>(p + 8 * g + 4 * hi) = v;
+  }
 }
 
 DEVI void philox_round(unsigned int& c0, unsigned int& c1,
@@ -136,8 +195,8 @@
 #pragma unroll
     for (int r = 0; r < 16; ++r)
       ot[j][r] *= alpha;
-  bf16x8 pf0 = assemble_pfrag(&s[0]);
-  bf16x8 pf1 = assemble_pfrag(&s[8]);
+  bf16x8 pf0 = assemble_pfrag<true>(&s[0]);
+  bf16x8 pf1 = assemble_pfrag<true>(&s[8]);
 #pragma unroll
   for (int kc = 0; kc < 2; ++kc) {
     bf16x8 pf = kc == 0 ? pf0 : pf1;
@@ -263,9 +322,7 @@
   short* op = out + (bh / heads) * o_sb + (bh % heads) * o_sh + myq * o_ss;
 #pragma unroll
   for (int j = 0; j < D / 32; ++j)
-#pragma unroll
-    for (int r = 0; r < 16; ++r)
-      op[j * 32 + crow(r, hi)] = (short)f2bf(ot[j][r] * inv_l);
+    store_acc_bf16(op + j * 32, ot[j] * inv_l, hi);
   if (hi == 0) lse[bh * seq + myq] = m + __logf(l);
 }
 
@@ -530,8 +587,112 @@
   }
 }
 
-template <bool DROP, bool DBUF, int D>
-__global__ __launch_bounds__(256, D == 64 ? (DBUF ? 3 : 4) : 2)
+template <bool MASKED, bool DROP, int D>
+DEVI void dv_tile_tr(const short* imgQ, const short* imgDO,
+                     const float* lseL, int sub, int64_t q0, int64_t seq,
+                     int64_t mykv, float scale, int causal,
+                     const bf16x8 (&kfrag)[D / 16], f32x16 (&dvt)[D / 32],
+                     int lkv, int hi, const unsigned int* maskrow,
+                     int64_t mask_w, float inv_keep) {
+  f32x16 st = load_rowconst(lseL, hi);
+#pragma unroll
+  for (int c = 0; c < D / 16; ++c) {
+    bf16x8 qf = *reinterpret_cast<const bf16x8*>(
+        imgQ + img_off<D>(sub + lkv, 2 * c + hi));
+    st = __builtin_amdgcn_mfma_f32_32x32x16_bf16(qf, kfrag[c], st, 0, 0, 0);
+  }
+  const float c2 = scale * 1.44269504088896341f;
+  const RowMask rm(q0, seq, mykv, causal);
+  float p[16];
+#pragma unroll
+  for (int r = 0; r < 16; ++r) {
+    if (MASKED)
+      p[r] = rm.masked(crow(r, hi)) ? 0.f
+                                    : __builtin_amdgcn_exp2f(st[r] * c2);
+    else
+      p[r] = __builtin_amdgcn_exp2f(st[r] * c2);
+    if (DROP) {
+      const int64_t qg = q0 + crow(r, hi);
+      const int64_t qgc = qg < seq ? qg : seq - 1;
+      const int64_t kvc = mykv < seq ? mykv : seq - 1;
+      const unsigned int w = maskrow[qgc * mask_w + (kvc >> 5)];
+      p[r] *= ((w >> (kvc & 31)) & 1u) ? inv_keep : 0.f;
+    }
+  }
+  bf16x8 pb0 = assemble_pfrag<true>(&p[0]);
+  bf16x8 pb1 = assemble_pfrag<true>(&p[8]);
+  const int lane = hi * 32 + lkv;
+#pragma unroll
+  for (int qc = 0; qc < 2; ++qc) {
+    bf16x8 pb = qc == 0 ? pb0 : pb1;
+#pragma unroll
+    for (int dj = 0; dj < D / 32; ++dj) {
+      bf16x8 dot = tr_frag<D>(imgDO, sub + qc * 16, dj, lane);
+      dvt[dj] =
+          __builtin_amdgcn_mfma_f32_32x32x16_bf16(dot, pb, dvt[dj], 0, 0, 0);
+    }
+  }
+}
+
+template <bool MASKED, bool DROP, int D>
+DEVI void dk_tile_tr(const short* imgQ, const short* imgDO,
+                     const float* lseL, const float* dltL, int sub,
+                     int64_t q0, int64_t seq, int64_t mykv, float scale,
+                     int causal, const bf16x8 (&kfrag)[D / 16],
+                     const bf16x8 (&vfrag)[D / 16], f32x16 (&dkt)[D / 32],
+                     int lkv, int hi, const unsigned int* maskrow,
+                     int64_t mask_w, float inv_keep) {
+  f32x16 st = load_rowconst(lseL, hi);
+  f32x16 dpt = {};
+  if (!DROP) dpt = load_rowconst(dltL, hi);
+#pragma unroll
+  for (int c = 0; c < D / 16; ++c) {
+    const int o = img_off<D>(sub + lkv, 2 * c + hi);
+    bf16x8 qf = *reinterpret_cast<const bf16x8*>(imgQ + o);
+    bf16x8 dof = *reinterpret_cast<const bf16x8*>(imgDO + o);
+    st = __builtin_amdgcn_mfma_f32_32x32x16_bf16(qf, kfrag[c], st, 0, 0, 0);
+    dpt = __builtin_amdgcn_mfma_f32_32x32x16_bf16(dof, vfrag[c], dpt, 0, 0,
+                                                  0);
+  }
+  const float c2 = scale * 1.44269504088896341f;
+  const RowMask rm(q0, seq, mykv, causal);
+  float ds[16];
+#pragma unroll
+  for (int r = 0; r < 16; ++r) {
+    float dp = dpt[r];
+    if (DROP) {
+      const int64_t qg = q0 + crow(r, hi);
+      const int64_t qgc = qg < seq ? qg : seq - 1;
+      const int64_t kvc = mykv < seq ? mykv : seq - 1;
+      const unsigned int w = maskrow[qgc * mask_w + (kvc >> 5)];
+      dp *= ((w >> (kvc & 31)) & 1u) ? inv_keep : 0.f;
+      dp += dltL[crow(r, hi)];
+    }
+    if (MASKED)
+      ds[r] = rm.masked(crow(r, hi))
+                  ? 0.f
+                  : __builtin_amdgcn_exp2f(st[r] * c2) * dp * scale;
+    else
+      ds[r] = __builtin_amdgcn_exp2f(st[r] * c2) * dp * scale;
+  }
+  bf16x8 db0 = assemble_pfrag<true>(&ds[0]);
+  bf16x8 db1 = assemble_pfrag<true>(&ds[8]);
+  const int lane = hi * 32 + lkv;
+#pragma unroll
+  for (int qc = 0; qc < 2; ++qc) {
+    bf16x8 db = qc == 0 ? db0 : db1;
+#pragma unroll
+    for (int dj = 0; dj < D / 32; ++dj) {
+      bf16x8 qt = tr_frag<D>(imgQ, sub + qc * 16, dj, lane);
+      dkt[dj] =
+          __builtin_amdgcn_mfma_f32_32x32x16_bf16(qt, db, dkt[dj], 0, 0, 0);
+    }
+  }
+}
+
+template <bool DROP, bool DBUF, int D, bool TR>
+__global__ __launch_bounds__(256, D == 64 ? (DBUF ? 3 : 4)
+                                          : (TR && !DROP ? 3 : 2))
 void attn_bwd_dv_kernel(
     const short* __restrict__ q, const short* __restrict__ k,
     const short* __restrict__ dout, const float* __restrict__ lse,
@@ -541,8 +702,12 @@
     int64_t g_sh, int64_t g_ss,
     const unsigned int* __restrict__ mask, int64_t mask_w,
     float inv_keep) {
-  __shared__ short ldsQ[DBUF ? 2 : 1][64][D + 8];
-  __shared__ short ldsDO[DBUF ? 2 : 1][64][D + 8];
+  constexpr int PITCH = TR ? img_pitch<D>() : D + 8;
+  __shared__ __attribute__((aligned(16))) short
+      ldsQ[DBUF ? 2 : 1][64][PITCH];
+  __shared__ __attribute__((aligned(16))) short
+      ldsDO[DBUF ? 2 : 1][64][PITCH];
+  __shared__ __attribute__((aligned(16))) float ldsL[DBUF ? 2 : 1][64];
   const int lane = threadIdx.x & 63;
   const int wave = threadIdx.x >> 6;
   const int hi = lane >> 5;
@@ -571,7 +736,13 @@
   const int stage_seg = (threadIdx.x & 7) * 8;
 
   bf16x8 rq[2][D / 64], rdo[2][D / 64];
+  float rl = 0.f;
+  const float neg_inv_scale = -1.f / scale;
   auto prefetch = [&](int64_t q0) {
+    if (TR && wave == 0) {
+      const int64_t qr = q0 + lane;
+      rl = lsep[qr < seq ? qr : seq - 1] * neg_inv_scale;
+    }
 #pragma unroll
     for (int half = 0; half < 2; ++half) {
       int64_t qr = q0 + stage_row + half * 32;
@@ -586,20 +757,27 @@
     }
   };
   auto commit = [&](int buf) {
+    if (TR && wave == 0) ldsL[buf][lane] = rl;
 #pragma unroll
     for (int half = 0; half < 2; ++half)
 #pragma unroll
       for (int s = 0; s < D / 64; ++s) {
         *reinterpret_cast<bf16x8*>(
-            &ldsQ[buf][stage_row + half * 32][stage_seg + s * 64]) =
+            img_at<TR, D>(ldsQ[buf], stage_row + half * 32,
+                          stage_seg + s * 64)) =
             rq[half][s];
         *reinterpret_cast<bf16x8*>(
-            &ldsDO[buf][stage_row + half * 32][stage_seg + s * 64]) =
+            img_at<TR, D>(ldsDO[buf], stage_row + half * 32,
+                          stage_seg + s * 64)) =
             rdo[half][s];
       }
   };
   auto stage_q64 = [&](int64_t q0) {
     __syncthreads();
+    if (TR && wave == 0) {
+      const int64_t qr = q0 + lane;
+      ldsL[0][lane] = lsep[qr < seq ? qr : seq - 1] * neg_inv_scale;
+    }
 #pragma unroll
     for (int half = 0; half < 2; ++half) {
       int64_t qr = q0 + stage_row + half * 32;
@@ -607,11 +785,13 @@
 #pragma unroll
       for (int seg = 0; seg < D; seg += 64) {
         *reinterpret_cast<bf16x8*>(
-            &ldsQ[0][stage_row + half * 32][stage_seg + seg]) =
+            img_at<TR, D>(ldsQ[0], stage_row + half * 32,
+                          stage_seg + seg)) =
             *reinterpret_cast<const bf16x8*>(
                 qp + qr * in_ss + stage_seg + seg);
         *reinterpret_cast<bf16x8*>(
-            &ldsDO[0][stage_row + half * 32][stage_seg + seg]) =
+            img_at<TR, D>(ldsDO[0], stage_row + half * 32,
+                          stage_seg + seg)) =
             *reinterpret_cast<const bf16x8*>(
                 dop + qr * do_ss + stage_seg + seg);
       }
@@ -621,6 +801,21 @@
 
   const unsigned int* maskrow =
       DROP ? mask + bh * seq * mask_w : (const unsigned int*)nullptr;
+  auto tile = [&](auto masked, int rb, int sub, int64_t q0s) {
+    constexpr bool M = decltype(masked)::value;
+    if constexpr (TR)
+      dv_tile_tr<M, DROP, D>(&ldsQ[rb][0][0], &ldsDO[rb][0][0],
+                             &ldsL[rb][sub], sub, q0s, seq, mykv, scale,
+                             causal, kfrag, dvt, lkv, hi, maskrow, mask_w,
+                             inv_keep);
+    else
+      dv_tile<M, DROP, D>(ldsQ[rb], ldsDO[rb], sub, q0s, seq, mykv, scale,
+                          causal, lsep, kfrag, dvt, lkv, hi, maskrow,
+                          mask_w, inv_keep);
+  };
+  constexpr std::true_type MASKED_T{};
+  constexpr std::false_type PLAIN_T{};
+
   const int64_t diag_end =
       causal ? (kv0_blk + 128 < seq ? kv0_blk + 128 : seq) : 0;
   const int64_t bulk_end = seq & ~(int64_t)63;
@@ -633,9 +828,7 @@
       for (int sub = 0; sub < 64; sub += 32) {
         const int64_t q0s = q0 + sub;
         if (q0s >= diag_end || (causal && q0s + 31 < kv0)) continue;
-        dv_tile<true, DROP, D>(ldsQ[0], ldsDO[0], sub, q0s, seq, mykv,
-                               scale, causal, lsep, kfrag, dvt, lkv, hi,
-                               maskrow, mask_w, inv_keep);
+        tile(MASKED_T, 0, sub, q0s);
       }
     }
     q0 = diag_end > q0 ? diag_end : q0;
@@ -643,9 +836,7 @@
       stage_q64(q0);
 #pragma unroll
       for (int sub = 0; sub < 64; sub += 32)
-        dv_tile<false, DROP, D>(ldsQ[0], ldsDO[0], sub, q0 + sub, seq,
-                                mykv, scale, causal, lsep, kfrag, dvt,
-                                lkv, hi, maskrow, mask_w, inv_keep);
+        tile(PLAIN_T, 0, sub, q0 + sub);
     }
     for (; q0 < seq; q0 += 64) {
       stage_q64(q0);
@@ -654,9 +845,7 @@
       for (int sub = 0; sub < 64; sub += 32) {
         const int64_t q0s = q0 + sub;
         if (q0s >= seq) break;
-        dv_tile<true, DROP, D>(ldsQ[0], ldsDO[0], sub, q0s, seq, mykv,
-                               scale, causal, lsep, kfrag, dvt, lkv, hi,
-                               maskrow, mask_w, inv_keep);
+        tile(MASKED_T, 0, sub, q0s);
       }
     }
   } else {
@@ -673,19 +862,14 @@
       if (plain) {
 #pragma unroll
         for (int sub = 0; sub < 64; sub += 32)
-          dv_tile<false, DROP, D>(ldsQ[rb], ldsDO[rb], sub, q0 + sub,
-                                  seq, mykv, scale, causal, lsep, kfrag,
-                                  dvt, lkv, hi, maskrow, mask_w,
-                                  inv_keep);
+          tile(PLAIN_T, rb, sub, q0 + sub);
       } else if (active) {
 #pragma unroll
         for (int sub = 0; sub < 64; sub += 32) {
           const int64_t q0s = q0 + sub;
           if (q0s >= seq) break;
           if (causal && q0s + 31 < kv0) continue;
-          dv_tile<true, DROP, D>(ldsQ[rb], ldsDO[rb], sub, q0s, seq,
-                                 mykv, scale, causal, lsep, kfrag, dvt,
-                                 lkv, hi, maskrow, mask_w, inv_keep);
+          tile(MASKED_T, rb, sub, q0s);
         }
       }
     }
@@ -694,13 +878,18 @@
   short* dvp = dv + (bh / heads) * g_sb + (bh % heads) * g_sh +
                mykv * g_ss;
 #pragma unroll
-  for (int dj = 0; dj < D / 32; ++dj)
-#pragma unroll
-    for (int r = 0; r < 16; ++r)
-      dvp[dj * 32 + crow(r, hi)] = (short)f2bf(dvt[dj][r]);
-}
-
-template <bool DROP, bool DBUF, int D>
+  for (int dj = 0; dj < D / 32; ++dj) {
+    if constexpr (TR) {
+      store_acc_bf16(dvp + dj * 32, dvt[dj], hi);
+    } else {
+#pragma unroll
+      for (int r = 0; r < 16; ++r)
+        dvp[dj * 32 + crow(r, hi)] = (short)f2bf(dvt[dj][r]);
+    }
+  }
+}
+
+template <bool DROP, bool DBUF, int D, bool TR>
 __global__ __launch_bounds__(256, D == 64 ? 3 : 2) void attn_bwd_dk_kernel(
     const short* __restrict__ q, const short* __restrict__ k,
     const short* __restrict__ v, const short* __restrict__ dout,
@@ -711,8 +900,12 @@
     int64_t g_sh, int64_t g_ss,
     const unsigned int* __restrict__ mask, int64_t mask_w,
     float inv_keep) {
-  __shared__ short ldsQ[DBUF ? 2 : 1][64][D + 8];
-  __shared__ short ldsDO[DBUF ? 2 : 1][64][D + 8];
+  constexpr int PITCH = TR ? img_pitch<D>() : D + 8;
+  __shared__ __attribute__((aligned(16))) short
+      ldsQ[DBUF ? 2 : 1][64][PITCH];
+  __shared__ __attribute__((aligned(16))) short
+      ldsDO[DBUF ? 2 : 1][64][PITCH];
+  __shared__ __attribute__((aligned(16))) float ldsL[DBUF ? 2 : 1][2][64];
   const int lane = threadIdx.x & 63;
   const int wave = threadIdx.x >> 6;
   const int hi = lane >> 5;
@@ -746,7 +939,14 @@
   const int stage_seg = (threadIdx.x & 7) * 8;
 
   bf16x8 rq[2][D / 64], rdo[2][D / 64];
+  float rl = 0.f;
+  const float neg_inv_scale = -1.f / scale;
   auto prefetch = [&](int64_t q0) {
+    if (TR && wave < 2) {
+      const int64_t qr = q0 + lane;
+      rl = (wave == 0 ? lsep : dltp)[qr < seq ? qr : seq - 1] *
+           (wave == 0 ? neg_inv_scale : -1.f);
+    }
 #pragma unroll
     for (int half = 0; half < 2; ++half) {
       int64_t qr = q0 + stage_row + half * 32;
@@ -761,20 +961,29 @@
     }
   };
   auto commit = [&](int buf) {
+    if (TR && wave < 2) ldsL[buf][wave][lane] = rl;
 #pragma unroll
     for (int half = 0; half < 2; ++half)
 #pragma unroll
       for (int s = 0; s < D / 64; ++s) {
         *reinterpret_cast<bf16x8*>(
-            &ldsQ[buf][stage_row + half * 32][stage_seg + s * 64]) =
+            img_at<TR, D>(ldsQ[buf], stage_row + half * 32,
+                          stage_seg + s * 64)) =
             rq[half][s];
         *reinterpret_cast<bf16x8*>(
-            &ldsDO[buf][stage_row + half * 32][stage_seg + s * 64]) =
+            img_at<TR, D>(ldsDO[buf], stage_row + half * 32,
+                          stage_seg + s * 64)) =
             rdo[half][s];
       }
   };
   auto stage_q64 = [&](int64_t q0) {
     __syncthreads();
+    if (TR && wave < 2) {
+      const int64_t qr = q0 + lane;
+      ldsL[0][wave][lane] =
+          (wave == 0 ? lsep : dltp)[qr < seq ? qr : seq - 1] *
+          (wave == 0 ? neg_inv_scale : -1.f);
+    }
 #pragma unroll
     for (int half = 0; half < 2; ++half) {
       int64_t qr = q0 + stage_row + half * 32;
@@ -782,11 +991,13 @@
 #pragma unroll
       for (int seg = 0; seg < D; seg += 64) {
         *reinterpret_cast<bf16x8*>(
-            &ldsQ[0][stage_row + half * 32][stage_seg + seg]) =
+            img_at<TR, D>(ldsQ[0], stage_row + half * 32,
+                          stage_seg + seg)) =
             *reinterpret_cast<const bf16x8*>(
                 qp + qr * in_ss + stage_seg + seg);
         *reinterpret_cast<bf16x8*>(
-            &ldsDO[0][stage_row + half * 32][stage_seg + seg]) =
+            img_at<TR, D>(ldsDO[0], stage_row + half * 32,
+                          stage_seg + seg)) =
             *reinterpret_cast<const bf16x8*>(
                 dop + qr * do_ss + stage_seg + seg);
       }
@@ -796,6 +1007,20 @@
 
   const unsigned int* maskrow =
       DROP ? mask + bh * seq * mask_w : (const unsigned int*)nullptr;
+  auto tile = [&](auto masked, int rb, int sub, int64_t q0s) {
+    constexpr bool M = decltype(masked)::value;
+    if constexpr (TR)
+      dk_tile_tr<M, DROP, D>(&ldsQ[rb][0][0], &ldsDO[rb][0][0],
+                             &ldsL[rb][0][sub], &ldsL[rb][1][sub], sub,
+                             q0s, seq, mykv, scale, causal, kfrag, vfrag,
+                             dkt, lkv, hi, maskrow, mask_w, inv_keep);
+    else
+      dk_tile<M, DROP, D>(ldsQ[rb], ldsDO[rb], sub, q0s, seq, mykv, scale,
+                          causal, lsep, dltp, kfrag, vfrag, dkt, lkv, hi,
+                          maskrow, mask_w, inv_keep);
+  };
+  constexpr std::true_type MASKED_T{};
+  constexpr std::false_type PLAIN_T{};
   const int64_t diag_end =
       causal ? (kv0_blk + 128 < seq ? kv0_blk + 128 : seq) : 0;
   const int64_t bulk_end = seq & ~(int64_t)63;
@@ -808,9 +1033,7 @@
       for (int sub = 0; sub < 64; sub += 32) {
         const int64_t q0s = q0 + sub;
         if (q0s >= diag_end || (causal && q0s + 31 < kv0)) continue;
-        dk_tile<true, DROP, D>(ldsQ[0], ldsDO[0], sub, q0s, seq, mykv,
-                               scale, causal, lsep, dltp, kfrag, vfrag,
-                               dkt, lkv, hi, maskrow, mask_w, inv_keep);
+        tile(MASKED_T, 0, sub, q0s);
       }
     }
     q0 = diag_end > q0 ? diag_end : q0;
@@ -818,10 +1041,7 @@
       stage_q64(q0);
 #pragma unroll
       for (int sub = 0; sub < 64; sub += 32)
-        dk_tile<false, DROP, D>(ldsQ[0], ldsDO[0], sub, q0 + sub, seq,
-                                mykv, scale, causal, lsep, dltp, kfrag,
-                                vfrag, dkt, lkv, hi, maskrow, mask_w,
-                                inv_keep);
+        tile(PLAIN_T, 0, sub, q0 + sub);
     }
     for (; q0 < seq; q0 += 64) {
       stage_q64(q0);
@@ -830,9 +1050,7 @@
       for (int sub = 0; sub < 64; sub += 32) {
         const int64_t q0s = q0 + sub;
         if (q0s >= seq) break;
-        dk_tile<true, DROP, D>(ldsQ[0], ldsDO[0], sub, q0s, seq, mykv,
-                               scale, causal, lsep, dltp, kfrag, vfrag,
-                               dkt, lkv, hi, maskrow, mask_w, inv_keep);
+        tile(MASKED_T, 0, sub, q0s);
       }
     }
   } else {
@@ -849,20 +1067,14 @@
       if (plain) {
 #pragma unroll
         for (int sub = 0; sub < 64; sub += 32)
-          dk_tile<false, DROP, D>(ldsQ[rb], ldsDO[rb], sub, q0 + sub,
-                                  seq, mykv, scale, causal, lsep, dltp,
-                                  kfrag, vfrag, dkt, lkv, hi, maskrow,
-                                  mask_w, inv_keep);
+          tile(PLAIN_T, rb, sub, q0 + sub);
       } else if (active) {
 #pragma unroll
         for (int sub = 0; sub < 64; sub += 32) {
           const int64_t q0s = q0 + sub;
           if (q0s >= seq) break;
           if (causal && q0s + 31 < kv0) continue;
-          dk_tile<true, DROP, D>(ldsQ[rb], ldsDO[rb], sub, q0s, seq,
-                                 mykv, scale, causal, lsep, dltp, kfrag,
-                                 vfrag, dkt, lkv, hi, maskrow, mask_w,
-                                 inv_keep);
+          tile(MASKED_T, rb, sub, q0s);
         }
       }
     }
@@ -871,10 +1083,15 @@
   short* dkp = dk + (bh / heads) * g_sb + (bh % heads) * g_sh +
                mykv * g_ss;
 #pragma unroll
-  for (int dj = 0; dj < D / 32; ++dj)
-#pragma unroll
-    for (int r = 0; r < 16; ++r)
-      dkp[dj * 32 + crow(r, hi)] = (short)f2bf(dkt[dj][r]);
+  for (int dj = 0; dj < D / 32; ++dj) {
+    if constexpr (TR) {
+      store_acc_bf16(dkp + dj * 32, dkt[dj], hi);
+    } else {
+#pragma unroll
+      for (int r = 0; r < 16; ++r)
+        dkp[dj * 32 + crow(r, hi)] = (short)f2bf(dkt[dj][r]);
+    }
+  }
 }
 
 
@@ -937,7 +1154,60 @@
   }
 }
 
-template <bool DROP, bool DBUF, int D>
+template <bool MASKED, bool DROP, int D>
+DEVI void dq_tile_tr(const short* imgK, const short* imgV, int sub,
+                     int64_t kv0, int64_t seq, int64_t myq, float scale,
+                     int causal, float mylse, float mydelta,
+                     const bf16x8 (&qfrag)[D / 16],
+                     const bf16x8 (&dofrag)[D / 16],
+                     f32x16 (&dqt)[D / 32], int lq, int hi,
+                     const unsigned int* maskrow, int64_t mask_w,
+                     float inv_keep) {
+  f32x16 st = {};
+  f32x16 dpt = {};
+#pragma unroll
+  for (int c = 0; c < D / 16; ++c) {
+    const int o = img_off<D>(sub + lq, 2 * c + hi);
+    bf16x8 kf = *reinterpret_cast<const bf16x8*>(imgK + o);
+    bf16x8 vf = *reinterpret_cast<const bf16x8*>(imgV + o);
+    st = __builtin_amdgcn_mfma_f32_32x32x16_bf16(kf, qfrag[c], st, 0, 0, 0);
+    dpt = __builtin_amdgcn_mfma_f32_32x32x16_bf16(vf, dofrag[c], dpt, 0, 0,
+                                                  0);
+  }
+  unsigned int mword = 0;
+  if (DROP) {
+    const int64_t qc = myq < seq ? myq : seq - 1;
+    mword = maskrow[qc * mask_w + (kv0 >> 5)];
+  }
+  float ds[16];
+#pragma unroll
+  for (int r = 0; r < 16; ++r) {
+    float pv = __expf(st[r] * scale - mylse);
+    if (MASKED) {
+      const int64_t kvg = kv0 + crow(r, hi);
+      if (myq >= seq || kvg >= seq || (causal && kvg > myq)) pv = 0.f;
+    }
+    float dp = dpt[r];
+    if (DROP)
+      dp *= ((mword >> crow(r, hi)) & 1u) ? inv_keep : 0.f;
+    ds[r] = pv * (dp - mydelta) * scale;
+  }
+  bf16x8 db0 = assemble_pfrag<true>(&ds[0]);
+  bf16x8 db1 = assemble_pfrag<true>(&ds[8]);
+  const int lane = hi * 32 + lq;
+#pragma unroll
+  for (int kc = 0; kc < 2; ++kc) {
+    bf16x8 db = kc == 0 ? db0 : db1;
+#pragma unroll
+    for (int dj = 0; dj < D / 32; ++dj) {
+      bf16x8 kt = tr_frag<D>(imgK, sub + kc * 16, dj, lane);
+      dqt[dj] =
+          __builtin_amdgcn_mfma_f32_32x32x16_bf16(kt, db, dqt[dj], 0, 0, 0);
+    }
+  }
+}
+
+template <bool DROP, bool DBUF, int D, bool TR>
 __global__ __launch_bounds__(256, D == 64 ? 3 : 2) void attn_bwd_dq_kernel(
     const short* __restrict__ q, const short* __restrict__ k,
     const short* __restrict__ v, const short* __restrict__ dout,
@@ -948,8 +1218,11 @@
     int64_t g_sb, int64_t g_sh, int64_t g_ss, int64_t o_sb, int64_t o_sh,
     int64_t o_ss, const unsigned int* __restrict__ mask, int64_t mask_w,
     float inv_keep, const float* __restrict__ dlse) {
-  __shared__ short ldsK[DBUF ? 2 : 1][64][D + 8];
-  __shared__ short ldsVr[DBUF ? 2 : 1][64][D + 8];
+  constexpr int PITCH = TR ? img_pitch<D>() : D + 8;
+  __shared__ __attribute__((aligned(16))) short
+      ldsK[DBUF ? 2 : 1][64][PITCH];
+  __shared__ __attribute__((aligned(16))) short
+      ldsVr[DBUF ? 2 : 1][64][PITCH];
   const int lane = threadIdx.x & 63;
   const int wave = threadIdx.x >> 6;
   const int hi = lane >> 5;
@@ -1007,11 +1280,13 @@
 #pragma unroll
       for (int seg = 0; seg < D; seg += 64) {
         *reinterpret_cast<bf16x8*>(
-            &ldsK[0][stage_row + half * 32][stage_seg + seg]) =
+            img_at<TR, D>(ldsK[0], stage_row + half * 32,
+                          stage_seg + seg)) =
             *reinterpret_cast<const bf16x8*>(
                 kp + kr * in_ss + stage_seg + seg);
         *reinterpret_cast<bf16x8*>(
-            &ldsVr[0][stage_row + half * 32][stage_seg + seg]) =
+            img_at<TR, D>(ldsVr[0], stage_row + half * 32,
+                          stage_seg + seg)) =
             *reinterpret_cast<const bf16x8*>(
                 vp + kr * in_ss + stage_seg + seg);
       }
@@ -1040,26 +1315,39 @@
 #pragma unroll
       for (int s = 0; s < D / 64; ++s) {
         *reinterpret_cast<bf16x8*>(
-            &ldsK[buf][stage_row + half * 32][stage_seg + s * 64]) =
+            img_at<TR, D>(ldsK[buf], stage_row + half * 32,
+                          stage_seg + s * 64)) =
             rk[half][s];
         *reinterpret_cast<bf16x8*>(
-            &ldsVr[buf][stage_row + half * 32][stage_seg + s * 64]) =
+            img_at<TR, D>(ldsVr[buf], stage_row + half * 32,
+                          stage_seg + s * 64)) =
             rv[half][s];
       }
   };
 
   const unsigned int* maskrow =
       DROP ? mask + bh * seq * mask_w : (const unsigned int*)nullptr;
+  auto tile = [&](auto masked, int rb, int sub, int64_t kvs) {
+    constexpr bool M = decltype(masked)::value;
+    if constexpr (TR)
+      dq_tile_tr<M, DROP, D>(&ldsK[rb][0][0], &ldsVr[rb][0][0], sub, kvs,
+                             seq, myq, scale, causal, mylse, mydelta,
+                             qfrag, dofrag, dqt, lq, hi, maskrow, mask_w,
+                             inv_keep);
+    else
+      dq_tile<M, DROP, D>(ldsK[rb], ldsVr[rb], sub, kvs, seq, myq, scale,
+                          causal, mylse, mydelta, qfrag, dofrag, dqt, lq,
+                          hi, maskrow, mask_w, inv_keep);
+  };
+  constexpr std::true_type MASKED_T{};
+  constexpr std::false_type PLAIN_T{};
   if (!DBUF) {
     int64_t kv0 = 0;
     for (; kv0 < bulk_end; kv0 += 64) {
       stage_kv64(kv0);
 #pragma unroll
       for (int sub = 0; sub < 64; sub += 32)
-        dq_tile<false, DROP, D>(ldsK[0], ldsVr[0], sub, kv0 + sub, seq,
-                                myq, scale, causal, mylse, mydelta,
-                                qfrag, dofrag, dqt, lq, hi, maskrow,
-                                mask_w, inv_keep);
+        tile(PLAIN_T, 0, sub, kv0 + sub);
     }
     for (; kv0 < blk_kv_end; kv0 += 64) {
       stage_kv64(kv0);
@@ -1070,10 +1358,7 @@
       for (int sub = 0; sub < 64; sub += 32) {
         const int64_t kvs = kv0 + sub;
         if (kvs >= wave_kv_end) break;
-        dq_tile<true, DROP, D>(ldsK[0], ldsVr[0], sub, kvs, seq, myq,
-                               scale, causal, mylse, mydelta, qfrag,
-                               dofrag, dqt, lq, hi, maskrow, mask_w,
-                               inv_keep);
+        tile(MASKED_T, 0, sub, kvs);
       }
     }
   } else {
@@ -1088,10 +1373,7 @@
       if (kv0 < bulk_end) {
 #pragma unroll
         for (int sub = 0; sub < 64; sub += 32)
-          dq_tile<false, DROP, D>(ldsK[rb], ldsVr[rb], sub, kv0 + sub,
-                                  seq, myq, scale, causal, mylse,
-                                  mydelta, qfrag, dofrag, dqt, lq, hi,
-                                  maskrow, mask_w, inv_keep);
+          tile(PLAIN_T, rb, sub, kv0 + sub);
       } else if (active) {
         const int64_t wave_kv_end = causal
             ? (q0 + 32 < seq ? q0 + 32 : seq) : seq;
@@ -1099,10 +1381,7 @@
         for (int sub = 0; sub < 64; sub += 32) {
           const int64_t kvs = kv0 + sub;
           if (kvs >= wave_kv_end) break;
-          dq_tile<true, DROP, D>(ldsK[rb], ldsVr[rb], sub, kvs, seq,
-                                 myq, scale, causal, mylse, mydelta,
-                                 qfrag, dofrag, dqt, lq, hi, maskrow,
-                                 mask_w, inv_keep);
+          tile(MASKED_T, rb, sub, kvs);
         }
       }
     }
@@ -1111,10 +1390,15 @@
   if (!active || myq >= seq) return;
   short* dqp = dq + (bh / heads) * g_sb + (bh % heads) * g_sh + myq * g_ss;
 #pragma unroll
-  for (int dj = 0; dj < D / 32; ++dj)
-#pragma unroll
-    for (int r = 0; r < 16; ++r)
-      dqp[dj * 32 + crow(r, hi)] = (short)f2bf(dqt[dj][r]);
+  for (int dj = 0; dj < D / 32; ++dj) {
+    if constexpr (TR) {
+      store_acc_bf16(dqp + dj * 32, dqt[dj], hi);
+    } else {
+#pragma unroll
+      for (int r = 0; r < 16; ++r)
+        dqp[dj * 32 + crow(r, hi)] = (short)f2bf(dqt[dj][r]);
+    }
+  }
 }
 
 }
@@ -1202,78 +1486,56 @@
     const bool dbuf = mode >= 1;
     const bool dbuf_k = mode >= 2;
     const bool dbuf_q = mode >= 3;
-    if (head_dim == 128) {
-      if (drop_mask != nullptr) {
+    static const bool legacy_tiles = [] {
+      const char* e = getenv("EPL_ATTN_BWD_TILES");
+      return e != nullptr && strcmp(e, "legacy") == 0;
+    }();
+    auto launch3 = [&](auto drop_c, auto d_c, auto tr_c) {
+      constexpr bool DROP = decltype(drop_c)::value;
+      constexpr int D = decltype(d_c)::value;
+      constexpr bool TR = decltype(tr_c)::value;
+      if (D == 64 && dbuf)
         hipLaunchKernelGGL(
-            HIP_KERNEL_NAME(attn_bwd_dv_kernel<true, false, 128>), grid,
-            dim3(256), 0, stream, DV_ARGS);
-        hipLaunchKernelGGL(
-            HIP_KERNEL_NAME(attn_bwd_dq_kernel<true, false, 128>), grid,
-            dim3(256), 0, stream, DQ_ARGS);
-        hipLaunchKernelGGL(
-            HIP_KERNEL_NAME(attn_bwd_dk_kernel<true, false, 128>), grid,
-            dim3(256), 0, stream, DK_ARGS);
-      } else {
-        hipLaunchKernelGGL(
-            HIP_KERNEL_NAME(attn_bwd_dv_kernel<false, false, 128>), grid,
-            dim3(256), 0, stream, DV_ARGS);
-        hipLaunchKernelGGL(
-            HIP_KERNEL_NAME(attn_bwd_dq_kernel<false, false, 128>), grid,
-            dim3(256), 0, stream, DQ_ARGS);
-        hipLaunchKernelGGL(
-            HIP_KERNEL_NAME(attn_bwd_dk_kernel<false, false, 128>), grid,
-            dim3(256), 0, stream, DK_ARGS);
-      }
-    } else if (drop_mask != nullptr) {
-      if (dbuf)
-        hipLaunchKernelGGL(
-            HIP_KERNEL_NAME(attn_bwd_dv_kernel<true, true, 64>), grid,
+            HIP_KERNEL_NAME(attn_bwd_dv_kernel<DROP, D == 64, D, TR>), grid,
             dim3(256), 0, stream, DV_ARGS);
       else
         hipLaunchKernelGGL(
-            HIP_KERNEL_NAME(attn_bwd_dv_kernel<true, false, 64>), grid,
+            HIP_KERNEL_NAME(attn_bwd_dv_kernel<DROP, false, D, TR>), grid,
             dim3(256), 0, stream, DV_ARGS);
-      if (dbuf_q)
+      if (D == 64 && dbuf_q)
         hipLaunchKernelGGL(
-            HIP_KERNEL_NAME(attn_bwd_dq_kernel<true, true, 64>), grid,
+            HIP_KERNEL_NAME(attn_bwd_dq_kernel<DROP, D == 64, D, TR>), grid,
             dim3(256), 0, stream, DQ_ARGS);
       else
         hipLaunchKernelGGL(
-            HIP_KERNEL_NAME(attn_bwd_dq_kernel<true, false, 64>), grid,
+            HIP_KERNEL_NAME(attn_bwd_dq_kernel<DROP, false, D, TR>), grid,
             dim3(256), 0, stream, DQ_ARGS);
-      if (dbuf_k)
+      if (D == 64 && dbuf_k)
         hipLaunchKernelGGL(
-            HIP_KERNEL_NAME(attn_bwd_dk_kernel<true, true, 64>), grid,
+            HIP_KERNEL_NAME(attn_bwd_dk_kernel<DROP, D == 64, D, TR>), grid,
             dim3(256), 0, stream, DK_ARGS);
       else
         hipLaunchKernelGGL(
-            HIP_KERNEL_NAME(attn_bwd_dk_kernel<true, false, 64>), grid,
+            HIP_KERNEL_NAME(attn_bwd_dk_kernel<DROP, false, D, TR>), grid,
             dim3(256), 0, stream, DK_ARGS);
+    };
+    auto launch2 = [&](auto drop_c, auto d_c) {
+      if (legacy_tiles)
+        launch3(drop_c, d_c, std::false_type{});
+      else
+        launch3(drop_c, d_c, std::true_type{});
+    };
+    using d64 = std::integral_constant<int, 64>;
+    using d128 = std::integral_constant<int, 128>;
+    if (head_dim == 128) {
+      if (drop_mask != nullptr)
+        launch2(std::true_type{}, d128{});
+      else
+        launch2(std::false_type{}, d128{});
+    } else if (drop_mask != nullptr) {
+      launch2(std::true_type{}, d64{});
     } else {
-      if (dbuf)
-        hipLaunchKernelGGL(
-            HIP_KERNEL_NAME(attn_bwd_dv_kernel<false, true, 64>), grid,
-            dim3(256), 0, stream, DV_ARGS);
-      else
-        hipLaunchKernelGGL(
-            HIP_KERNEL_NAME(attn_bwd_dv_kernel<false, false, 64>), grid,
-            dim3(256), 0, stream, DV_ARGS);
-      if (dbuf_q)
-        hipLaunchKernelGGL(
-            HIP_KERNEL_NAME(attn_bwd_dq_kernel<false, true, 64>), grid,
-            dim3(256), 0, stream, DQ_ARGS);
-      else
-        hipLaunchKernelGGL(
-            HIP_KERNEL_NAME(attn_bwd_dq_kernel<false, false, 64>), grid,
-            dim3(256), 0, stream, DQ_ARGS);
-      if (dbuf_k)
-        hipLaunchKernelGGL(
-            HIP_KERNEL_NAME(attn_bwd_dk_kernel<false, true, 64>), grid,
-            dim3(256), 0, stream, DK_ARGS);
-      else
-        hipLaunchKernelGGL(
-            HIP_KERNEL_NAME(attn_bwd_dk_kernel<false, false, 64>), grid,
-            dim3(256), 0, stream, DK_ARGS);
+      launch2(std::false_type{}, d64{});
     }
 #undef DV_ARGS
 #undef DQ_ARGS
@@ -1302,7 +1564,8 @@
                      in_strides[2], do_strides[0], do_strides[1],
                      do_strides[2], g_strides[0], g_strides[1],
                      g_strides[2]);
-  hipLaunchKernelGGL(HIP_KERNEL_NAME(attn_bwd_dq_kernel<false, false, 64>),
+  hipLaunchKernelGGL(
+      HIP_KERNEL_NAME(attn_bwd_dq_kernel<false, false, 64, true>),
                      grid, dim3(256), 0, stream,
                      reinterpret_cast<const short*>(q),
                      reinterpret_cast<const short*>(k),
diff --git a/csrc/kernels/attn_lds_image.h b/csrc/kernels/attn_lds_image.h
--- /dev/null
+++ b/csrc/kernels/attn_lds_image.h
@@ -0,0 +1,43 @@
+#pragma once
+
+#include <hip/hip_runtime.h>
+
+namespace attn_img {
+
+using s16x4 = __attribute__((ext_vector_type(4))) short;
+using s16x8 = __attribute__((ext_vector_type(8))) short;
+
+template <int D>
+constexpr int img_pitch() { return D == 64 ? 72 : 152; }
+
+template <int D>
+__device__ __forceinline__ int img_off(int row, int ch) {
+  return row * img_pitch<D>() + 8 * ch;
+}
+
+template <int D>
+__device__ __forceinline__ s16x8 tr_frag(const short* img, int r0, int dj,
+                                         int lane) {
+  typedef s16x4 __attribute__((address_space(3))) lds_b64;
+  const int row = r0 + 8 * (lane >> 5) + ((lane & 15) >> 2);
+  const int ch = 4 * dj + 2 * ((lane >> 4) & 1) + ((lane & 3) >> 1);
+  const int sub = 4 * (lane & 1);
+  s16x4 lo = __builtin_amdgcn_ds_read_tr16_b64_v4i16(
+      (lds_b64*)(img + img_off<D>(row, ch) + sub));
+  s16x4 hi4 = __builtin_amdgcn_ds_read_tr16_b64_v4i16(
+      (lds_b64*)(img + img_off<D>(row + 4, ch) + sub));
+  return __builtin_shufflevector(lo, hi4, 0, 1, 2, 3, 4, 5, 6, 7);
+}
+
+template <int D>
+__device__ __forceinline__ s16x8 gather_frag(const short* img, int r0,
+                                             int dj, int lane) {
+  s16x8 out;
+  const int col = 32 * dj + (lane & 31);
+#pragma unroll
+  for (int j = 0; j < 8; ++j)
+    out[j] = img[img_off<D>(r0 + 8 * (lane >> 5) + j, col >> 3) + (col & 7)];
+  return out;
+}
+
+}
diff --git a/csrc/kernels/mfma_probe.hip b/csrc/kernels/mfma_probe.hip
--- a/csrc/kernels/mfma_probe.hip
+++ b/csrc/kernels/mfma_probe.hip
@@ -1,5 +1,7 @@
 
 #include <hip/hip_runtime.h>
+
+#include "attn_lds_image.h"
 
 using bf16x8 = __attribute__((ext_vector_type(8))) short;
 using f32x16 = __attribute__((ext_vector_type(16))) float;
@@ -30,3 +32,37 @@
   hipLaunchKernelGGL(mfma_probe_kernel, dim3(1), dim3(64), 0, stream, A, B,
                      D);
 }
+
+template <int D>
+__global__ void tr_read_probe_kernel(short* __restrict__ out_gather,
+                                     short* __restrict__ out_tr) {
+  __shared__ __attribute__((aligned(16))) short
+      img[64 * attn_img::img_pitch<D>()];
+  const int lane = threadIdx.x & 63;
+  for (int i = lane; i < 64 * D; i += 64) {
+    const int row = i / D, col = i % D;
+    img[attn_img::img_off<D>(row, col >> 3) + (col & 7)] =
+        (short)(row * 256 + col);
+  }
+  __syncthreads();
+  for (int sub = 0; sub < 64; sub += 32)
+    for (int qc = 0; qc < 2; ++qc)
+      for (int dj = 0; dj < D / 32; ++dj) {
+        const int frag = ((sub >> 5) * 2 + qc) * (D / 32) + dj;
+        const bf16x8 g =
+            attn_img::gather_frag<D>(img, sub + qc * 16, dj, lane);
+        const bf16x8 t = attn_img::tr_frag<D>(img, sub + qc * 16, dj, lane);
+        *reinterpret_cast<bf16x8*>(out_gather + (frag * 64 + lane) * 8) = g;
+        *reinterpret_cast<bf16x8*>(out_tr + (frag * 64 + lane) * 8) = t;
+      }
+}
+
+extern "C" void run_tr_read_probe(short* out_gather, short* out_tr,
+                                  int head_dim, hipStream_t stream) {
+  if (head_dim == 128)
+    hipLaunchKernelGGL(tr_read_probe_kernel<128>, dim3(1), dim3(64), 0,
+                       stream, out_gather, out_tr);
+  else
+    hipLaunchKernelGGL(tr_read_probe_kernel<64>, dim3(1), dim3(64), 0,
+                       stream, out_gather, out_tr);
+}
```
